# VisionDepth/VisionDepth3D

Hardware: AMD Instinct MI355X
Metric: stereo-pairs/sec end-to-end (depth+warp+fill+mux) (higher is better)
Workload: dtype f32; 1 GPU; 4k-dav2b-dibr; frame=3840x2160, format=Half-SBS, depth_model=depth-anything-v2-base, depth_net_dtype=float32 (the reference's precision), pixel_overlap=True, pixel_streams=2, clip_frames_all_ranks=32, params=render_cli.py defaults + dof_strength 2.0, dense DOF order (parity mode)

## Files before the change

include/vd3d.h:

```cpp
#ifndef VD3D_H
#define VD3D_H

#include <stddef.h>
#include <stdint.h>

#ifdef __cplusplus
extern "C" {
#endif

#define VD3D_ABI_VERSION 6

typedef enum vd3d_status {
  VD3D_OK = 0,
  VD3D_E_INVALID = -1,
  VD3D_E_HIP = -2,
  VD3D_E_NOMEM = -3,
  VD3D_E_UNSUPPORTED = -4
} vd3d_status;

typedef enum vd3d_format {
  VD3D_FMT_HALF_SBS = 0,
  VD3D_FMT_FULL_SBS = 1,
  VD3D_FMT_VR = 2,
  VD3D_FMT_ANAGLYPH = 3,
// ... 117 lines not shown

int vd3d_render_frame_blank(vd3d_ctx* ctx, const uint8_t* frame_bgr, const void* depth, int depth_fmt,
                            const vd3d_render_params* p, uint8_t* out_bgr);

int vd3d_shard_begin(vd3d_ctx* ctx, const vd3d_render_params* p, int n_slots);
int vd3d_shard_pixels(vd3d_ctx* ctx, int slot, const vd3d_render_params* p, uint8_t* out_bgr);
int vd3d_shard_pixels_blank(vd3d_ctx* ctx, int slot, const uint8_t* frame_bgr, const vd3d_render_params* p, uint8_t* out_bgr);
int vd3d_set_pixel_overlap(vd3d_ctx* ctx, int enable);
int vd3d_join_pixels(vd3d_ctx* ctx);
int vd3d_wait_pixels(vd3d_ctx* ctx, int slot);

int vd3d_shard2_p0(vd3d_ctx* ctx, const uint8_t* frame_bgr, const vd3d_render_params* p, int* crop_out_dev);
int vd3d_shard2_set_crops(vd3d_ctx* ctx, const int* crops_all_dev, int n);
int vd3d_shard2_p1(vd3d_ctx* ctx, const uint8_t* frame_bgr, const void* depth, int depth_fmt,
                   const vd3d_render_params* p, int step_idx, int slot, float* q_out_dev);
int vd3d_tdf_plane_export(vd3d_ctx* ctx, float* dst_dev, int eye_h, int eye_w);
int vd3d_tdf_plane_import(vd3d_ctx* ctx, const float* src_dev, int eye_h, int eye_w, int valid);
int vd3d_shard2_r1(vd3d_ctx* ctx, const float* q_all_dev, int n);
int vd3d_shard2_p3(vd3d_ctx* ctx, int slot, int step_idx, const vd3d_render_params* p, long long* m_out_dev);
int vd3d_shard2_p1_batch(vd3d_ctx* ctx, const uint8_t* const* frames_bgr, const void* const* depths, int depth_fmt,
                         const vd3d_render_params* p, int step_idx0, int slot0, int n, float* q_out_dev);
int vd3d_shard2_p3_batch(vd3d_ctx* ctx, int slot0, int step_idx0, int n, const vd3d_render_params* p, long long* m_out_dev);
int vd3d_shard2_r2(vd3d_ctx* ctx, const long long* m_all_dev, const int* own_slot_host, const uint8_t* blank_host_or_null, int n,
                   const vd3d_render_params* p);

int vd3d_heal_missing_pixels(vd3d_ctx* ctx, const float* warped_chw, const float* original_chw, const float* edge_mask_or_null,
                             int H, int W, double heal_strength, float* out_chw);

int vd3d_nv12_to_bgr(vd3d_ctx* ctx, const uint8_t* y_plane, long long y_pitch, const uint8_t* uv_plane, long long uv_pitch, int h, int w,
                     uint8_t* out_bgr);
int vd3d_bgr_to_nv12(vd3d_ctx* ctx, const uint8_t* bgr, int h, int w, uint8_t* y_plane, long long y_pitch, uint8_t* uv_plane,
                     long long uv_pitch);

int vd3d_resize_cubic_u8(vd3d_ctx* ctx, const uint8_t* src, int sh, int sw, int cn, uint8_t* dst, int dh, int dw);
int vd3d_resize_area_u8(vd3d_ctx* ctx, const uint8_t* src_bgr, int sh, int sw, uint8_t* dst_bgr, int dh, int dw);
int vd3d_resize_linear_u8(vd3d_ctx* ctx, const uint8_t* src_bgr, int sh, int sw, uint8_t* dst_bgr, int dh, int dw);
int vd3d_format_3d_output(vd3d_ctx* ctx, const uint8_t* left_bgr, const uint8_t* right_bgr, int h, int w, int format, uint8_t* out_bgr);

int vd3d_esr_preprocess(vd3d_ctx* ctx, int dtype, const uint8_t* frame_bgr, long long pitch_bytes, int h, int w, int channels_last,
                        void* out_rgb);
int vd3d_esr_postprocess(vd3d_ctx* ctx, const float* pred_rgb, int h, int w, int channels_last, int cy, int cx, int ch, int cw,
                         uint8_t* out_bgr, long long pitch_bytes);
int vd3d_add_weighted_u8(vd3d_ctx* ctx, const uint8_t* a, double alpha, const uint8_t* b, double beta, double gamma, long long n,
                         uint8_t* out);
int vd3d_rife_preprocess(vd3d_ctx* ctx, int dtype, const uint8_t* frame1_bgr, const uint8_t* frame2_bgr, int h, int w, int channels_last,
                         void* out6);
int vd3d_rife_postprocess(vd3d_ctx* ctx, const float* pred3, int h, int w, int channels_last, uint8_t* out_bgr);

int vd3d_conv3x3_c64_f16(vd3d_ctx* ctx, const void* x_nhwc, int H, int W, const void* w_frag, const float* bias, const float* slope_or_null,
                         void* y_nhwc);
int vd3d_conv3x3_head_f16(vd3d_ctx* ctx, const void* x_nhwc3, int H, int W, const float* w27x64, const float* bias, const float* slope_or_null,
                          void* y_nhwc64);
int vd3d_esr_tail_f32(vd3d_ctx* ctx, const void* t_nhwc64, const void* x_nhwc3, int H, int W, int r, float* out_planar);
int vd3d_conv3x3_dense_f16(vd3d_ctx* ctx, const void* x, int H, int W, int x_stride, int Cin, const void* w_frag, const float* bias, int Cout,
                           float slope, float alpha, const void* r1_or_null, int r1_stride, float beta, const void* r2_or_null, int r2_stride,
                           int up2, void* y, int y_stride, int y_offset);
int vd3d_nhwc_f16_to_planar3_f32(vd3d_ctx* ctx, const void* t_nhwc32, int H, int W, float* out_planar);

int vd3d_depth_handoff(vd3d_ctx* ctx, const float* pred, int B, int ph, int pw, int H, int W, int invert, uint8_t* out_gray);
int vd3d_depth_handoff_form(vd3d_ctx* ctx, const float* pred, int B, int ph, int pw, int H, int W, int invert, uint8_t* out_gray, int form);

int vd3d_tile_gather_cubic_u8(vd3d_ctx* ctx, const uint8_t* frames_bgr, long long pitch_bytes, long long frame_stride_bytes, int B, int H, int W,
                              const int32_t* origins_dev, int n, int ch, int cw, int chs, int cws, uint8_t* out_tiles);
int vd3d_tile_blend_f32(vd3d_ctx* ctx, const float* pred_pool, const int64_t* pred_off_dev, const int32_t* tile_tab_dev, const float* w_pool,
                        int B, int tgt_h, int tgt_w, int tile, int pad, float* out);
int vd3d_depth_normalize_pclip_u8(vd3d_ctx* ctx, const float* planes, int B, int H, int W, float p_lo, float p_hi, int invert, uint8_t* out_gray,
                                  float* lo_hi_dev_or_null);

typedef struct vd3d_letterbox_state {
  int32_t top, bottom;
  int32_t locked_zero, locked_bars;
  int32_t cand_top, cand_bottom, streak;
  int32_t cooldown;
  int32_t have_prev, prev_h, prev_w;
  int32_t reserved;
} vd3d_letterbox_state;
typedef struct vd3d_letterbox_params {
  int32_t min_change, confirm_needed;
  int32_t max_total;
  int32_t cooldown_frames;
} vd3d_letterbox_params;
int vd3d_letterbox_stats(vd3d_ctx* ctx, const uint8_t* frames_bgr, int B, int H, int W, int chain, float* row_mean, float* row_var,
                         uint32_t* row_sat_sum, uint8_t* gray, uint32_t* hist64, uint64_t* mad_sum, float* frame_mean);
int vd3d_canny_u8(vd3d_ctx* ctx, const uint8_t* gray, int B, int H, int W, int low, int high, uint8_t* edges, int32_t* row_counts_or_null);
int vd3d_canny_hysteresis_u8(vd3d_ctx* ctx, const uint8_t* classes, int B, int H, int W, uint8_t* edges, int32_t* row_counts_or_null);
int vd3d_letterbox_track(vd3d_ctx* ctx, const uint8_t* frames_bgr, int B, int H, int W, const vd3d_letterbox_params* params, int32_t* out_bars);
int vd3d_letterbox_state_reset(vd3d_ctx* ctx);
int vd3d_letterbox_state_export(vd3d_ctx* ctx, vd3d_letterbox_state* out, uint32_t* prev_hist64_host_or_null, uint8_t* prev_gray_dev_or_null,
                                long long gray_capacity);
int vd3d_letterbox_state_import(vd3d_ctx* ctx, const vd3d_letterbox_state* in, const uint32_t* prev_hist64_host_or_null,
                                const uint8_t* prev_gray_dev_or_null);
int vd3d_depth_letterbox_fill_u8(vd3d_ctx* ctx, const uint8_t* depth, int B, int H, int W, const int32_t* bars_dev, int bars_stride, uint8_t* out);

typedef enum vd3d_dtype { VD3D_DT_BF16 = 0, VD3D_DT_F32 = 1, VD3D_DT_F16 = 2  } vd3d_dtype;

int vd3d_depth_preprocess(vd3d_ctx* ctx, const uint8_t* frames_bgr, int B, int H, int W, int th, int tw,
                          const float* mean3_host, const float* std3_host, int dtype, void* out_nhwc);
int vd3d_depth_preprocess_form(vd3d_ctx* ctx, const uint8_t* frames_bgr, int B, int H, int W, int th, int tw,
                               const float* mean3_host, const float* std3_host, int dtype, void* out_nhwc, int form);

int vd3d_resize_pil_bicubic_u8(vd3d_ctx* ctx, const uint8_t* src, int B, int H, int W, uint8_t* dst, int h, int w);
int vd3d_depth_preprocess_pil(vd3d_ctx* ctx, const uint8_t* frames_bgr, int B, int H, int W, int mid_h, int mid_w, int th, int tw,
                              const float* mean3_host, const float* std3_host, int dtype, void* out_nhwc);

int vd3d_add_layernorm(vd3d_ctx* ctx, int dtype, const void* x, const void* y_or_null, const void* gamma, const void* beta,
                       float eps, int64_t rows, int cols, void* out_sum, void* out_norm);

enum { VD3D_GEMM_EPI_NONE = 0, VD3D_GEMM_EPI_GELU = 1 };
enum { VD3D_X3_BF16X3 = 0, VD3D_X3_FP16X2 = 1 };
int64_t vd3d_gemm_x3_weight_bytes(int N, int K, int mode);
int vd3d_gemm_x3_pack_weights(vd3d_ctx* ctx, const float* W, int N, int K, int mode, void* image);
int vd3d_gemm_x3(vd3d_ctx* ctx, const float* X, int64_t M, int K, const void* w_image, int N, int mode, const float* bias_or_null, int epilogue, float* Y);
int64_t vd3d_attention_x3_workspace_bytes(int B, int T, int H, int D, int mode);
int vd3d_attention_x3(vd3d_ctx* ctx, const float* qkv, int B, int T, int H, int D, float scale, int mode, void* workspace, int64_t workspace_bytes, float* out);
int vd3d_attention_f32(vd3d_ctx* ctx, const float* qkv, int B, int T, int H, int D, float scale, float* out);
int vd3d_attention_f32_form(vd3d_ctx* ctx, const float* qkv, int B, int T, int H, int D, float scale, float* out, int form);

int64_t vd3d_conv3x3_x2_weight_bytes(int Cin, int Cout);
int vd3d_conv3x3_x2_pack_weights(vd3d_ctx* ctx, const float* W, int Cin, int Cout, void* image);
int vd3d_conv3x3_x2(vd3d_ctx* ctx, const float* X, int B, int H, int W, int Cin, const void* w_image, int Cout, float* Y);
int64_t vd3d_conv3x3_x3_weight_bytes(int Cin, int Cout);
int vd3d_conv3x3_x3_pack_weights(vd3d_ctx* ctx, const float* W, int Cin, int Cout, void* image);
int vd3d_conv3x3_x3(vd3d_ctx* ctx, const float* X, int B, int H, int W, int Cin, const void* w_image, int Cout, float* Y);
int64_t vd3d_conv3x3_s2_x3_weight_bytes(int Cin, int Cout);
int vd3d_conv3x3_s2_x3_pack_weights(vd3d_ctx* ctx, const float* W, int Cin, int Cout, void* image);
int vd3d_conv3x3_s2_x3(vd3d_ctx* ctx, const float* X, int B, int H, int W, int Cin, const void* w_image, int Cout, float* Y);
int64_t vd3d_conv3x3_s1_x2_weight_bytes(int Cin, int Cout);
int vd3d_conv3x3_s1_x2_pack_weights(vd3d_ctx* ctx, const float* W, int Cin, int Cout, void* image);
int vd3d_conv3x3_s1_x2(vd3d_ctx* ctx, const float* X, int B, int H, int W, int Cin, const void* w_image, int Cout, float* Y);
int64_t vd3d_conv3x3_s2_x2_weight_bytes(int Cin, int Cout);
int vd3d_conv3x3_s2_x2_pack_weights(vd3d_ctx* ctx, const float* W, int Cin, int Cout, void* image);
int vd3d_conv3x3_s2_x2(vd3d_ctx* ctx, const float* X, int B, int H, int W, int Cin, const void* w_image, int Cout, float* Y);

enum { VD3D_IFN_K3S1 = 0, VD3D_IFN_K3S2 = 1, VD3D_IFN_T4S2 = 2 };
int64_t vd3d_conv_ifn_weight_bytes(int kind, int Cin, int Cout);
int vd3d_conv_ifn_pack_weights(vd3d_ctx* ctx, int kind, const float* W, int Cin, int Cout, void* image);
int vd3d_conv_ifn(vd3d_ctx* ctx, int kind, const float* X, int B, int H, int W, int x_stride, int Cin, const void* w_image, const float* bias,
                  const float* slope_or_null, int Cout, const float* r_or_null, int r_stride, float* Y, int y_stride, int y_offset);
int vd3d_rife_warp_pack(vd3d_ctx* ctx, const float* x6, const float* state_or_null, int N, int h, int w, int scale, float* out16);
int vd3d_rife_update(vd3d_ctx* ctx, const float* t, int t_stride, int first, int N, int h, int w, int scale, float* state);
int vd3d_rife_blend(vd3d_ctx* ctx, const float* x6, const float* state, int N, int h, int w, float* out);

int vd3d_upsample_bilinear_nhwc(vd3d_ctx* ctx, int dtype, const void* in, void* out, int B, int ih, int iw, int oh, int ow, int C);

int vd3d_nhwc_bias_act_f32(vd3d_ctx* ctx, const float* y, const float* bias_or_null, const float* r1_or_null, const float* r2_or_null, int relu,
                           int64_t n_pix, int C, float* out, float* relu_out_or_null);
int vd3d_upsample_bilinear_bias_nhwc_f32(vd3d_ctx* ctx, const float* in, const float* bias, float* out, int B, int ih, int iw, int oh, int ow, int C);
int vd3d_dpt_head_tail_f32(vd3d_ctx* ctx, const float* y, const float* b2, const float* w3, float b3, float scale, int64_t n_pix, int C, float* out);

int64_t vd3d_dpt_head_conv_weight_bytes(int Cin, int Cout);
int vd3d_dpt_head_conv_pack_weights(vd3d_ctx* ctx, const float* W, int Cin, int Cout, void* image);
int vd3d_dpt_head_conv_f32(vd3d_ctx* ctx, const float* x, const float* b_in, int B, int ih, int iw, int oh, int ow, int Cin, const void* w_image, int Cout,
                           const float* b2_or_null, const float* w3_or_null, float b3, float scale, float* out);

int vd3d_depth_to_space_bias_nhwc_f32(vd3d_ctx* ctx, const float* y, const float* bias_or_null, int B, int H, int W, int s, int C, float* out);

int vd3d_patchify_f32(vd3d_ctx* ctx, const float* x, int B, int th, int tw, int p, float* rows);

typedef enum vd3d_preview {
  VD3D_PREVIEW_INTERLACED = 0,
  VD3D_PREVIEW_HSBS = 1,
  VD3D_PREVIEW_LR_DIFF = 2,
  VD3D_PREVIEW_FEATHER_BLEND = 3,
  VD3D_PREVIEW_RED_BLUE = 4
} vd3d_preview;
int vd3d_preview_image(vd3d_ctx* ctx, int type, const uint8_t* left_bgr, const uint8_t* right_bgr, int h, int w, uint8_t* out_bgr);
int vd3d_preview_heatmap(vd3d_ctx* ctx, int type, const float* shift_map, int h, int w, const uint8_t* lut_bgr_dev, uint8_t* out_bgr);
int vd3d_preview_arrows(vd3d_ctx* ctx, const uint8_t* left_bgr, const float* shift_map, int h, int w, uint8_t* out_bgr);

int vd3d_finish_frame(vd3d_ctx* ctx, const uint8_t* left_bgr, const uint8_t* right_bgr,
                      const float* depth_norm, int eye_h, int eye_w,
                      const vd3d_render_params* p, double focal_depth, int bar_width, int bar_side,
                      uint8_t* out_bgr);
int vd3d_quantiles(vd3d_ctx* ctx, const float* plane, int64_t n, const float* q_host, int nq, float* out_host);
int vd3d_subject_depth(vd3d_ctx* ctx, const float* plane, int H, int W, float* out_host);
int vd3d_detect_black_bars(vd3d_ctx* ctx, const uint8_t* frame_bgr, int h, int w, int* top_host, int* bottom_host);
int vd3d_stream_copy(vd3d_ctx* ctx, const void* src, void* dst, size_t bytes);
int vd3d_torch_math(vd3d_ctx* ctx, int op, const float* x, float param, float* out, long long n);
int vd3d_torch_math_aten(vd3d_ctx* ctx, int op, const float* x, double param, float* out, long long n, int aten_threads);
int vd3d_set_profiling(vd3d_ctx* ctx, int enable);
int vd3d_debug_tune(int which, int value);
float vd3d_last_stage_ms(vd3d_ctx* ctx, const char* stage);
long vd3d_stage_calls(vd3d_ctx* ctx, const char* stage);
int vd3d_debug_gaussian_kernel1d(int k, float sigma, float* out_host);
int vd3d_debug_exp_torch(const float* x_host, float* out_host, long long n);
int vd3d_debug_planes(vd3d_ctx* ctx, float** D, float** S, uint8_t** L, uint8_t** R, float** rgb_eye, float** dn_cur);

#ifdef __cplusplus
}
#endif
#endif
```

visiondepth3d_amd/_lib.py:

```python
from __future__ import annotations

import ctypes as C
import os

from . import _abi
from ._abi import FrameScalars, LetterboxParams, LetterboxState, RenderParams, ShiftParams, State

_HERE = os.path.dirname(os.path.abspath(__file__))
LIB_PATH = os.environ.get("VD3D_LIB_PATH") or os.path.join(_HERE, "libvd3d_hip.so")

EXPORTS = (
    "vd3d_abi_version", "vd3d_last_error", "vd3d_shift_params_default", "vd3d_render_params_default",
    "vd3d_ctx_create", "vd3d_ctx_destroy", "vd3d_sync", "vd3d_ctx_stream", "vd3d_ctx_set_stream", "vd3d_ctx_pixel_stream", "vd3d_ctx_pixel_stream_k",
    "vd3d_state_reset", "vd3d_state_new_clip", "vd3d_state_export", "vd3d_state_import", "vd3d_state_planes",
    "vd3d_last_scalars", "vd3d_pixel_shift", "vd3d_render_frame", "vd3d_render_frame_blank", "vd3d_depth_handoff", "vd3d_depth_handoff_form", "vd3d_heal_missing_pixels", "vd3d_preview_heatmap", "vd3d_preview_arrows", "vd3d_conv3x3_c64_f16", "vd3d_conv3x3_head_f16", "vd3d_esr_tail_f32", "vd3d_conv3x3_dense_f16", "vd3d_nhwc_f16_to_planar3_f32", "vd3d_nv12_to_bgr", "vd3d_bgr_to_nv12", "vd3d_resize_cubic_u8", "vd3d_resize_area_u8", "vd3d_resize_linear_u8", "vd3d_format_3d_output", "vd3d_esr_preprocess", "vd3d_esr_postprocess", "vd3d_add_weighted_u8", "vd3d_rife_preprocess", "vd3d_rife_postprocess",
    "vd3d_shard_begin", "vd3d_shard_pixels", "vd3d_shard_pixels_blank", "vd3d_tdf_plane_export", "vd3d_tdf_plane_import", "vd3d_set_pixel_overlap", "vd3d_join_pixels", "vd3d_wait_pixels", "vd3d_finish_frame", "vd3d_quantiles",
    "vd3d_subject_depth", "vd3d_shard2_p0", "vd3d_shard2_set_crops", "vd3d_shard2_p1", "vd3d_shard2_p1_batch", "vd3d_shard2_r1", "vd3d_shard2_p3", "vd3d_shard2_p3_batch", "vd3d_shard2_r2", "vd3d_depth_preprocess", "vd3d_depth_preprocess_form", "vd3d_resize_pil_bicubic_u8", "vd3d_depth_preprocess_pil", "vd3d_tile_gather_cubic_u8", "vd3d_tile_blend_f32", "vd3d_depth_normalize_pclip_u8", "vd3d_letterbox_stats", "vd3d_canny_u8", "vd3d_canny_hysteresis_u8", "vd3d_letterbox_track", "vd3d_letterbox_state_reset", "vd3d_letterbox_state_export", "vd3d_letterbox_state_import", "vd3d_depth_letterbox_fill_u8", "vd3d_add_layernorm", "vd3d_gemm_x3_weight_bytes", "vd3d_gemm_x3_pack_weights", "vd3d_gemm_x3", "vd3d_attention_x3_workspace_bytes", "vd3d_attention_x3", "vd3d_attention_f32", "vd3d_attention_f32_form", "vd3d_conv3x3_x2_weight_bytes", "vd3d_conv3x3_x2_pack_weights", "vd3d_conv3x3_x2", "vd3d_conv3x3_x3_weight_bytes", "vd3d_conv3x3_x3_pack_weights", "vd3d_conv3x3_x3", "vd3d_conv3x3_s2_x3_weight_bytes", "vd3d_conv3x3_s2_x3_pack_weights", "vd3d_conv3x3_s2_x3", "vd3d_conv3x3_s1_x2_weight_bytes", "vd3d_conv3x3_s1_x2_pack_weights", "vd3d_conv3x3_s1_x2", "vd3d_conv3x3_s2_x2_weight_bytes", "vd3d_conv3x3_s2_x2_pack_weights", "vd3d_conv3x3_s2_x2", "vd3d_conv_ifn_weight_bytes", "vd3d_conv_ifn_pack_weights", "vd3d_conv_ifn", "vd3d_rife_warp_pack", "vd3d_rife_update", "vd3d_rife_blend", "vd3d_upsample_bilinear_nhwc", "vd3d_nhwc_bias_act_f32", "vd3d_upsample_bilinear_bias_nhwc_f32", "vd3d_dpt_head_tail_f32", "vd3d_dpt_head_conv_weight_bytes", "vd3d_dpt_head_conv_pack_weights", "vd3d_dpt_head_conv_f32", "vd3d_depth_to_space_bias_nhwc_f32", "vd3d_patchify_f32", "vd3d_preview_image", "vd3d_detect_black_bars", "vd3d_stream_copy", "vd3d_torch_math", "vd3d_torch_math_aten", "vd3d_debug_gaussian_kernel1d", "vd3d_debug_exp_torch", "vd3d_set_profiling", "vd3d_last_stage_ms", "vd3d_stage_calls",
    "vd3d_debug_planes", "vd3d_debug_tune",
)

_lib = None


class Vd3dError(RuntimeError):
    def __init__(self, code, msg):
        super().__init__(f"libvd3d_hip error {code}: {msg}")
        self.code = code


def lib():
    global _lib
    if _lib is not None:
        return _lib
    if not os.path.exists(LIB_PATH):
        raise ImportError(f"{LIB_PATH} not built: run `python -c 'import __graft_entry__ as g; g.build()'` "
                          "(hipcc --offload-arch=gfx950). There is no CPU fallback.")
    L = C.CDLL(LIB_PATH)
    vp, i32, f32p, u8p = C.c_void_p, C.c_int, C.c_void_p, C.c_void_p
    L.vd3d_abi_version.restype = i32
    L.vd3d_last_error.restype = C.c_char_p
    L.vd3d_ctx_create.argtypes = [i32, vp, C.POINTER(vp)]
    L.vd3d_ctx_destroy.argtypes = [vp]
    L.vd3d_sync.argtypes = [vp]
    L.vd3d_ctx_stream.argtypes = [vp]
    L.vd3d_ctx_stream.restype = vp
    L.vd3d_ctx_set_stream.argtypes = [vp, vp]
    L.vd3d_ctx_pixel_stream.argtypes = [vp]
    L.vd3d_ctx_pixel_stream.restype = vp
    L.vd3d_ctx_pixel_stream_k.argtypes = [vp, i32]
    L.vd3d_ctx_pixel_stream_k.restype = vp
    for n in ("vd3d_state_reset", "vd3d_state_new_clip"):
        getattr(L, n).argtypes = [vp]
    L.vd3d_state_export.argtypes = [vp, C.POINTER(State)]
    L.vd3d_state_import.argtypes = [vp, C.POINTER(State)]
    L.vd3d_state_planes.argtypes = [vp, C.POINTER(vp), C.POINTER(vp), C.POINTER(i32), C.POINTER(i32)]
    L.vd3d_last_scalars.argtypes = [vp, C.POINTER(FrameScalars)]
    L.vd3d_pixel_shift.argtypes = [vp, f32p, f32p, i32, i32, i32, i32, C.POINTER(ShiftParams), u8p, u8p, f32p]
    L.vd3d_render_frame.argtypes = [vp, u8p, vp, i32, C.POINTER(RenderParams), u8p]
    L.vd3d_render_frame_blank.argtypes = [vp, u8p, vp, i32, C.POINTER(RenderParams), u8p]
    L.vd3d_shard_begin.argtypes = [vp, C.POINTER(RenderParams), i32]
    L.vd3d_shard_pixels.argtypes = [vp, i32, C.POINTER(RenderParams), u8p]
    L.vd3d_shard_pixels_blank.argtypes = [vp, i32, u8p, C.POINTER(RenderParams), u8p]
    L.vd3d_tdf_plane_export.argtypes = [vp, f32p, i32, i32]
    L.vd3d_tdf_plane_import.argtypes = [vp, f32p, i32, i32, i32]
    L.vd3d_set_pixel_overlap.argtypes = [vp, i32]
    L.vd3d_join_pixels.argtypes = [vp]
    L.vd3d_wait_pixels.argtypes = [vp, i32]
    L.vd3d_depth_handoff.argtypes = [vp, f32p, i32, i32, i32, i32, i32, i32, u8p]
    L.vd3d_depth_handoff_form.argtypes = [vp, f32p, i32, i32, i32, i32, i32, i32, u8p, i32]
    L.vd3d_heal_missing_pixels.argtypes = [vp, f32p, f32p, f32p, i32, i32, C.c_double, f32p]
    L.vd3d_resize_cubic_u8.argtypes = [vp, u8p, i32, i32, i32, u8p, i32, i32]
    L.vd3d_nv12_to_bgr.argtypes = [vp, u8p, C.c_longlong, u8p, C.c_longlong, i32, i32, u8p]
    L.vd3d_bgr_to_nv12.argtypes = [vp, u8p, i32, i32, u8p, C.c_longlong, u8p, C.c_longlong]
    L.vd3d_conv3x3_c64_f16.argtypes = [vp, vp, i32, i32, vp, vp, vp, vp]
    L.vd3d_conv3x3_head_f16.argtypes = [vp, vp, i32, i32, vp, vp, vp, vp]
    L.vd3d_esr_tail_f32.argtypes = [vp, vp, vp, i32, i32, i32, vp]
    L.vd3d_conv3x3_dense_f16.argtypes = [vp, vp, i32, i32, i32, i32, vp, vp, i32, C.c_float, C.c_float, vp, i32, C.c_float, vp, i32, i32, vp, i32, i32]
    L.vd3d_nhwc_f16_to_planar3_f32.argtypes = [vp, vp, i32, i32, vp]
    L.vd3d_preview_arrows.argtypes = [vp, u8p, f32p, i32, i32, u8p]
    L.vd3d_preview_heatmap.argtypes = [vp, i32, f32p, i32, i32, u8p, u8p]
    L.vd3d_resize_area_u8.argtypes = [vp, u8p, i32, i32, u8p, i32, i32]
    L.vd3d_resize_linear_u8.argtypes = [vp, u8p, i32, i32, u8p, i32, i32]
    L.vd3d_format_3d_output.argtypes = [vp, u8p, u8p, i32, i32, i32, u8p]
    L.vd3d_esr_preprocess.argtypes = [vp, i32, u8p, C.c_longlong, i32, i32, i32, vp]
    L.vd3d_esr_postprocess.argtypes = [vp, f32p, i32, i32, i32, i32, i32, i32, i32, u8p, C.c_longlong]
    L.vd3d_rife_preprocess.argtypes = [vp, i32, u8p, u8p, i32, i32, i32, vp]
    L.vd3d_rife_postprocess.argtypes = [vp, f32p, i32, i32, i32, u8p]
    L.vd3d_add_weighted_u8.argtypes = [vp, u8p, C.c_double, u8p, C.c_double, C.c_double, C.c_longlong, u8p]
    L.vd3d_finish_frame.argtypes = [vp, u8p, u8p, f32p, i32, i32, C.POINTER(RenderParams), C.c_double, i32, i32, u8p]
    L.vd3d_quantiles.argtypes = [vp, f32p, C.c_int64, C.POINTER(C.c_float), i32, C.POINTER(C.c_float)]
    L.vd3d_subject_depth.argtypes = [vp, f32p, i32, i32, C.POINTER(C.c_float)]
    L.vd3d_shard2_p0.argtypes = [vp, vp, vp, vp]
    L.vd3d_shard2_set_crops.argtypes = [vp, vp, i32]
    L.vd3d_shard2_p1.argtypes = [vp, vp, vp, i32, vp, i32, i32, vp]
    L.vd3d_shard2_p1_batch.argtypes = [vp, vp, vp, i32, vp, i32, i32, i32, vp]
    L.vd3d_shard2_p3_batch.argtypes = [vp, i32, i32, i32, vp, vp]
    L.vd3d_shard2_r1.argtypes = [vp, vp, i32]
    L.vd3d_shard2_p3.argtypes = [vp, i32, i32, vp, vp]
    L.vd3d_shard2_r2.argtypes = [vp, vp, C.POINTER(C.c_int), C.POINTER(C.c_uint8), i32, vp]
    L.vd3d_depth_preprocess.argtypes = [vp, vp, i32, i32, i32, i32, i32, C.POINTER(C.c_float), C.POINTER(C.c_float), i32, vp]
    L.vd3d_depth_preprocess_form.argtypes = [vp, vp, i32, i32, i32, i32, i32, C.POINTER(C.c_float), C.POINTER(C.c_float), i32, vp, i32]
    L.vd3d_resize_pil_bicubic_u8.argtypes = [vp, u8p, i32, i32, i32, u8p, i32, i32]
    L.vd3d_depth_preprocess_pil.argtypes = [vp, vp, i32, i32, i32, i32, i32, i32, i32, C.POINTER(C.c_float), C.POINTER(C.c_float), i32, vp]
    L.vd3d_tile_gather_cubic_u8.argtypes = [vp, u8p, C.c_longlong, C.c_longlong, i32, i32, i32, vp, i32, i32, i32, i32, i32, u8p]
    L.vd3d_tile_blend_f32.argtypes = [vp, f32p, vp, vp, f32p, i32, i32, i32, i32, i32, f32p]
    L.vd3d_depth_normalize_pclip_u8.argtypes = [vp, f32p, i32, i32, i32, C.c_float, C.c_float, i32, u8p, f32p]
    L.vd3d_letterbox_stats.argtypes = [vp, u8p, i32, i32, i32, i32, f32p, f32p, vp, u8p, vp, vp, f32p]
    L.vd3d_canny_u8.argtypes = [vp, u8p, i32, i32, i32, i32, i32, u8p, vp]
    L.vd3d_canny_hysteresis_u8.argtypes = [vp, u8p, i32, i32, i32, u8p, vp]
    L.vd3d_letterbox_track.argtypes = [vp, u8p, i32, i32, i32, C.POINTER(LetterboxParams), vp]
    L.vd3d_letterbox_state_reset.argtypes = [vp]
    L.vd3d_letterbox_state_export.argtypes = [vp, C.POINTER(LetterboxState), vp, u8p, C.c_longlong]
    L.vd3d_letterbox_state_import.argtypes = [vp, C.POINTER(LetterboxState), vp, u8p]
    L.vd3d_depth_letterbox_fill_u8.argtypes = [vp, u8p, i32, i32, i32, vp, i32, u8p]
    L.vd3d_gemm_x3_weight_bytes.argtypes = [i32, i32, i32]
    L.vd3d_gemm_x3_weight_bytes.restype = C.c_int64
    L.vd3d_gemm_x3_pack_weights.argtypes = [vp, vp, i32, i32, i32, vp]
    L.vd3d_gemm_x3.argtypes = [vp, vp, C.c_int64, i32, vp, i32, i32, vp, i32, vp]
    L.vd3d_attention_x3_workspace_bytes.argtypes = [i32, i32, i32, i32, i32]
    L.vd3d_attention_x3_workspace_bytes.restype = C.c_int64
    L.vd3d_attention_x3.argtypes = [vp, vp, i32, i32, i32, i32, C.c_float, i32, vp, C.c_int64, vp]
    L.vd3d_attention_f32.argtypes = [vp, vp, i32, i32, i32, i32, C.c_float, vp]
    L.vd3d_attention_f32_form.argtypes = [vp, vp, i32, i32, i32, i32, C.c_float, vp, i32]
    L.vd3d_conv3x3_x2_weight_bytes.argtypes = [i32, i32]
    L.vd3d_conv3x3_x2_weight_bytes.restype = C.c_int64
    L.vd3d_conv3x3_x2_pack_weights.argtypes = [vp, vp, i32, i32, vp]
    L.vd3d_conv3x3_x2.argtypes = [vp, vp, i32, i32, i32, i32, vp, i32, vp]
    L.vd3d_conv3x3_x3_weight_bytes.argtypes = [i32, i32]
    L.vd3d_conv3x3_x3_weight_bytes.restype = C.c_int64
    L.vd3d_conv3x3_x3_pack_weights.argtypes = [vp, vp, i32, i32, vp]
    L.vd3d_conv3x3_x3.argtypes = [vp, vp, i32, i32, i32, i32, vp, i32, vp]
    L.vd3d_conv3x3_s2_x3_weight_bytes.argtypes = [i32, i32]
    L.vd3d_conv3x3_s2_x3_weight_bytes.restype = C.c_int64
    L.vd3d_conv3x3_s2_x3_pack_weights.argtypes = [vp, vp, i32, i32, vp]
    L.vd3d_conv3x3_s2_x3.argtypes = [vp, vp, i32, i32, i32, i32, vp, i32, vp]
    for st in ("s1", "s2"):
        getattr(L, f"vd3d_conv3x3_{st}_x2_weight_bytes").argtypes = [i32, i32]
        getattr(L, f"vd3d_conv3x3_{st}_x2_weight_bytes").restype = C.c_int64
        getattr(L, f"vd3d_conv3x3_{st}_x2_pack_weights").argtypes = [vp, vp, i32, i32, vp]
        getattr(L, f"vd3d_conv3x3_{st}_x2").argtypes = [vp, vp, i32, i32, i32, i32, vp, i32, vp]
    L.vd3d_conv_ifn_weight_bytes.argtypes = [i32, i32, i32]
    L.vd3d_conv_ifn_weight_bytes.restype = C.c_int64
    L.vd3d_conv_ifn_pack_weights.argtypes = [vp, i32, vp, i32, i32, vp]
    L.vd3d_conv_ifn.argtypes = [vp, i32, vp, i32, i32, i32, i32, i32, vp, vp, vp, i32, vp, i32, vp, i32, i32]
    L.vd3d_rife_warp_pack.argtypes = [vp, vp, vp, i32, i32, i32, i32, vp]
    L.vd3d_rife_update.argtypes = [vp, vp, i32, i32, i32, i32, i32, i32, vp]
    L.vd3d_rife_blend.argtypes = [vp, vp, vp, i32, i32, i32, vp]
    L.vd3d_add_layernorm.argtypes = [vp, i32, vp, vp, vp, vp, C.c_float, C.c_int64, i32, vp, vp]
    L.vd3d_upsample_bilinear_nhwc.argtypes = [vp, i32, vp, vp, i32, i32, i32, i32, i32, i32]
    L.vd3d_nhwc_bias_act_f32.argtypes = [vp, vp, vp, vp, vp, i32, C.c_int64, i32, vp, vp]
    L.vd3d_upsample_bilinear_bias_nhwc_f32.argtypes = [vp, vp, vp, vp, i32, i32, i32, i32, i32, i32]
    L.vd3d_dpt_head_tail_f32.argtypes = [vp, vp, vp, vp, C.c_float, C.c_float, C.c_int64, i32, vp]
    L.vd3d_dpt_head_conv_weight_bytes.argtypes = [i32, i32]
    L.vd3d_dpt_head_conv_weight_bytes.restype = C.c_int64
    L.vd3d_dpt_head_conv_pack_weights.argtypes = [vp, vp, i32, i32, vp]
    L.vd3d_dpt_head_conv_f32.argtypes = [vp, vp, vp, i32, i32, i32, i32, i32, i32, vp, i32, vp, vp, C.c_float, C.c_float, vp]
    L.vd3d_depth_to_space_bias_nhwc_f32.argtypes = [vp, vp, vp, i32, i32, i32, i32, i32, vp]
    L.vd3d_patchify_f32.argtypes = [vp, vp, i32, i32, i32, i32, vp]
    L.vd3d_preview_image.argtypes = [vp, i32, vp, vp, i32, i32, vp]
    L.vd3d_detect_black_bars.argtypes = [vp, vp, i32, i32, C.POINTER(C.c_int), C.POINTER(C.c_int)]
    L.vd3d_stream_copy.argtypes = [vp, vp, vp, C.c_size_t]
    L.vd3d_torch_math.argtypes = [vp, i32, vp, C.c_float, vp, C.c_longlong]
    L.vd3d_torch_math_aten.argtypes = [vp, i32, vp, C.c_double, vp, C.c_longlong, i32]
    L.vd3d_debug_gaussian_kernel1d.argtypes = [i32, C.c_float, vp]
    L.vd3d_debug_exp_torch.argtypes = [vp, vp, C.c_longlong]
    L.vd3d_debug_tune.argtypes = [i32, i32]
    L.vd3d_set_profiling.argtypes = [vp, i32]
    L.vd3d_last_stage_ms.argtypes = [vp, C.c_char_p]
    L.vd3d_last_stage_ms.restype = C.c_float
    L.vd3d_stage_calls.argtypes = [vp, C.c_char_p]
    L.vd3d_stage_calls.restype = C.c_long
    L.vd3d_debug_planes.argtypes = [vp] + [C.POINTER(vp)] * 6
    L.vd3d_shift_params_default.argtypes = [C.POINTER(ShiftParams)]
    L.vd3d_render_params_default.argtypes = [C.POINTER(RenderParams)]
    if L.vd3d_abi_version() != _abi.ABI_VERSION:
        raise ImportError("libvd3d_hip.so ABI version mismatch")
    if os.environ.get("VD3D_TUNE"):
        if L.vd3d_debug_tune(-1, 0) != 0:
            raise ImportError("VD3D_TUNE is set but this libvd3d_hip.so was built without -DVD3D_DEV_KNOBS (bash tools/build_ab.sh dev -DVD3D_DEV_KNOBS; VD3D_LIB_PATH=...)")
        for kv in filter(None, os.environ["VD3D_TUNE"].split(",")):
            k, v = kv.split(":")
            if L.vd3d_debug_tune(int(k), int(v)) != 0:
                raise ImportError(f"VD3D_TUNE: unknown knob {k}")
    _lib = L
    return L


def check(rc):
    if rc != 0:
        raise Vd3dError(rc, lib().vd3d_last_error().decode(errors="replace"))
```

visiondepth3d_amd/csrc/vd3d_api.hip:

```cpp
#include <hip/hip_runtime.h>

#include <cmath>
#include <cstdarg>
#include <cstddef>
#include <cstdio>
#include <cstring>
#include <cstdlib>
#include <list>
#include <map>
#include <string>
#include <vector>

#include "vd3d_kernels.h"

#define VD3D_EXPORT extern "C" __attribute__((visibility("default")))

static thread_local char g_err[512] = "";
static int set_err(int code, const char* fmt, ...) {
  va_list ap;
  va_start(ap, fmt);
  vsnprintf(g_err, sizeof g_err, fmt, ap);
  va_end(ap);
  return code;
}
// ... 1693 lines not shown
    return set_err(VD3D_E_UNSUPPORTED, "conv_ifn: bias, slope, residual and output must be 4-byte aligned");
  const int Ho = kind == VD3D_IFN_K3S2 ? (H + 1) / 2 : kind == VD3D_IFN_T4S2 ? 2 * H : H, Wo = kind == VD3D_IFN_K3S2 ? (W + 1) / 2 : kind == VD3D_IFN_T4S2 ? 2 * W : W;
  {
    const long long in_pix = (long long)B * H * W, out_pix = (long long)B * Ho * Wo;
    const uintptr_t xb = (uintptr_t)X, xe = xb + (uintptr_t)(((in_pix - 1) * x_stride + Cin) * 4);
    const uintptr_t yb = (uintptr_t)Y + (uintptr_t)y_offset * 4, ye = (uintptr_t)Y + (uintptr_t)(((out_pix - 1) * y_stride + y_offset + Cout) * 4);
    const bool same_grid = (const void*)X == (const void*)Y && x_stride == y_stride && kind == VD3D_IFN_K3S1;
    if (same_grid ? y_offset < Cin : (xb < ye && yb < xe))
      return set_err(VD3D_E_UNSUPPORTED, "conv_ifn: the output slice [%d, %d) meets the input channels [0, %d) of the same buffer (a race between workgroups)",
                     y_offset, y_offset + Cout, Cin);
    if (r_or_null) {
      const uintptr_t rb = (uintptr_t)r_or_null, re = rb + (uintptr_t)(((out_pix - 1) * r_stride + Cout) * 4);
      const bool rgrid = (const void*)r_or_null == (const void*)Y && r_stride == y_stride;
      if (rgrid ? y_offset < Cout : (rb < ye && yb < re)) return set_err(VD3D_E_UNSUPPORTED, "conv_ifn: the residual overlaps the output slice");
    }
  }
  HIPCHK(hipSetDevice(c->device));
  StageTimer t(c, "conv_ifn");
  if (!vd_launch_conv_ifn(c->stream, kind, X, B, H, W, x_stride, Cin, w_image, bias, slope_or_null, Cout, r_or_null, r_stride, Y, y_stride, y_offset))
    return set_err(VD3D_E_HIP, "conv_ifn: the dynamic LDS opt-in failed");
  HIPCHK(hipGetLastError());
  return 0;
}

static int rife_glue_err(const char* what, int N, int h, int w, int scale) {
  return set_err(VD3D_E_UNSUPPORTED, "%s: N %d must be 1 .. 65535, the frame %d x %d 1 .. 32768 on each side, scale %d one of 1, 2, 4 and every pointer 16-byte aligned", what, N, h, w, scale);
}
static bool rife_glue_ok(int N, int h, int w, int scale) { return N >= 1 && N <= 65535 && h >= 1 && w >= 1 && h <= 32768 && w <= 32768 && (scale == 1 || scale == 2 || scale == 4); }

VD3D_EXPORT int vd3d_rife_warp_pack(vd3d_ctx* c, const float* x6, const float* state_or_null, int N, int h, int w, int scale, float* out16) {
  if (!c || !x6 || !out16) return set_err(VD3D_E_INVALID, "rife_warp_pack: null argument");
  if (!rife_glue_ok(N, h, w, scale) || (((uintptr_t)x6 | (uintptr_t)state_or_null | (uintptr_t)out16) & 15)) return rife_glue_err("rife_warp_pack", N, h, w, scale);
  HIPCHK(hipSetDevice(c->device));
  StageTimer t(c, "rife_glue");
  vd_launch_rife_warp_pack(c->stream, x6, state_or_null, state_or_null ? 0 : 1, N, h, w, (h + 31) / 32 * 32, (w + 31) / 32 * 32, scale, out16);
  HIPCHK(hipGetLastError());
  return 0;
}

VD3D_EXPORT int vd3d_rife_update(vd3d_ctx* c, const float* t_, int t_stride, int first, int N, int h, int w, int scale, float* state) {
  if (!c || !t_ || !state) return set_err(VD3D_E_INVALID, "rife_update: null argument");
  if (!rife_glue_ok(N, h, w, scale) || (((uintptr_t)t_ | (uintptr_t)state) & 15)) return rife_glue_err("rife_update", N, h, w, scale);
  if (t_stride < 5 || (t_stride & 3)) return set_err(VD3D_E_UNSUPPORTED, "rife_update: t_stride %d must be a multiple of 4 and >= 5", t_stride);
  HIPCHK(hipSetDevice(c->device));
  StageTimer t(c, "rife_glue");
  vd_launch_rife_update(c->stream, t_, t_stride, first ? 1 : 0, N, (h + 31) / 32 * 32, (w + 31) / 32 * 32, scale, state);
  HIPCHK(hipGetLastError());
  return 0;
}

VD3D_EXPORT int vd3d_rife_blend(vd3d_ctx* c, const float* x6, const float* state, int N, int h, int w, float* out) {
  if (!c || !x6 || !state || !out) return set_err(VD3D_E_INVALID, "rife_blend: null argument");
  if (!rife_glue_ok(N, h, w, 1) || (((uintptr_t)x6 | (uintptr_t)state | (uintptr_t)out) & 15)) return rife_glue_err("rife_blend", N, h, w, 1);
  HIPCHK(hipSetDevice(c->device));
  StageTimer t(c, "rife_glue");
  vd_launch_rife_blend(c->stream, x6, state, N, h, w, (h + 31) / 32 * 32, (w + 31) / 32 * 32, out);
  HIPCHK(hipGetLastError());
  return 0;
}

VD3D_EXPORT int64_t vd3d_attention_x3_workspace_bytes(int B, int T, int H, int D, int mode) { return (int64_t)vd_attn_x3_workspace_bytes(B, T, H, D, mode); }

VD3D_EXPORT int vd3d_attention_x3(vd3d_ctx* c, const float* qkv, int B, int T, int H, int D, float scale, int mode, void* workspace, int64_t workspace_bytes, float* out) {
  if (!c || !qkv || !workspace || !out) return set_err(VD3D_E_INVALID, "bad argument");
  const long long need = vd_attn_x3_workspace_bytes(B, T, H, D, mode);
  if (need < 0) return set_err(VD3D_E_UNSUPPORTED, "attention_x3: head size %d not built (64), an unknown mode %d or an empty shape (B %d T %d H %d)", D, mode, B, T, H);
  if (workspace_bytes < need) return set_err(VD3D_E_INVALID, "attention_x3: workspace of %lld bytes, %lld needed", (long long)workspace_bytes, need);
  HIPCHK(hipSetDevice(c->device));
  if (!vd_launch_attn_x3(c->stream, qkv, B, T, H, D, scale, workspace, out, mode))
    return set_err(VD3D_E_UNSUPPORTED, "attention_x3: qkv / workspace / out must be 16-byte aligned, B * H <= 65535");
  HIPCHK(hipGetLastError());
  return 0;
}

VD3D_EXPORT int vd3d_attention_f32_form(vd3d_ctx* c, const float* qkv, int B, int T, int H, int D, float scale, float* out, int form) {
  if (!c || !qkv || !out) return set_err(VD3D_E_INVALID, "bad argument");
  if (form != 0 && form != 4 && form != 8) return set_err(VD3D_E_INVALID, "attention_f32: form %d is not 0 (choose), 4 or 8 waves per workgroup", form);
  HIPCHK(hipSetDevice(c->device));
  if (!vd_launch_attn_f32(c->stream, qkv, B, T, H, D, scale, out, form))
    return set_err(VD3D_E_UNSUPPORTED, "attention_f32: head size %d not built (64), an empty shape (B %d T %d H %d), B * H > 65535 or qkv / out not 16-byte aligned", D, B, T, H);
  HIPCHK(hipGetLastError());
  return 0;
}

VD3D_EXPORT int vd3d_attention_f32(vd3d_ctx* c, const float* qkv, int B, int T, int H, int D, float scale, float* out) {
  return vd3d_attention_f32_form(c, qkv, B, T, H, D, scale, out, 0);
}

VD3D_EXPORT int64_t vd3d_gemm_x3_weight_bytes(int N, int K, int mode) { return (int64_t)vd_gemm_x3_weight_bytes(N, K, mode); }

VD3D_EXPORT int vd3d_gemm_x3_pack_weights(vd3d_ctx* c, const float* W, int N, int K, int mode, void* image) {
  if (!c || !W || !image) return set_err(VD3D_E_INVALID, "bad argument");
  HIPCHK(hipSetDevice(c->device));
  if (!vd_launch_gemm_x3_pack_w(c->stream, W, N, K, image, mode)) return set_err(VD3D_E_UNSUPPORTED, "gemm_x3: K %d must be a positive multiple of 16 (N %d), mode %d in {0, 1}", K, N, mode);
  HIPCHK(hipGetLastError());
  return 0;
}

VD3D_EXPORT int vd3d_gemm_x3(vd3d_ctx* c, const float* X, int64_t M, int K, const void* w_image, int N, int mode, const float* bias_or_null, int epilogue, float* Y) {
  if (!c || !X || !w_image || !Y || M < 1) return set_err(VD3D_E_INVALID, "bad argument");
  if (epilogue != VD3D_GEMM_EPI_NONE && epilogue != VD3D_GEMM_EPI_GELU) return set_err(VD3D_E_INVALID, "gemm_x3: unknown epilogue %d", epilogue);
  HIPCHK(hipSetDevice(c->device));
  if (!vd_launch_gemm_x3(c->stream, X, (long long)M, K, w_image, N, bias_or_null, epilogue, Y, mode))
    return set_err(VD3D_E_UNSUPPORTED, "gemm_x3: K %d must be a positive multiple of 16, mode %d in {0, 1}, X and the weight image 16-byte aligned", K, mode);
  HIPCHK(hipGetLastError());
  return 0;
}

VD3D_EXPORT int vd3d_upsample_bilinear_nhwc(vd3d_ctx* c, int dtype, const void* in, void* out, int B, int ih, int iw, int oh, int ow, int C) {
  if (dtype != VD3D_DT_BF16 && dtype != VD3D_DT_F32) return set_err(VD3D_E_INVALID, "bad dtype %d", dtype);
  if (!c || !in || !out || B < 1 || ih < 1 || iw < 1) return set_err(VD3D_E_INVALID, "bad argument");
  if (!vd_launch_upsample_bilinear_nhwc(c->stream, dtype, in, out, B, ih, iw, oh, ow, C))
    return set_err(VD3D_E_UNSUPPORTED, "upsample_bilinear_nhwc: C not a multiple of 8 (bf16) / 4 (f32) or output smaller than 2x2");
  HIPCHK(hipGetLastError());
  return 0;
}

VD3D_EXPORT int vd3d_nhwc_bias_act_f32(vd3d_ctx* c, const float* y, const float* bias_or_null, const float* r1_or_null, const float* r2_or_null, int relu,
                                       int64_t n_pix, int C, float* out, float* relu_out_or_null) {
  if (!c || !y || !out || n_pix < 1 || C < 4) return set_err(VD3D_E_INVALID, "bad argument");
  HIPCHK(hipSetDevice(c->device));
  if (!vd_launch_bias_act_f32(c->stream, y, bias_or_null, r1_or_null, r2_or_null, relu, (long long)n_pix, C, out, relu_out_or_null))
    return set_err(VD3D_E_UNSUPPORTED, "nhwc_bias_act: C %d not a multiple of 4", C);
  HIPCHK(hipGetLastError());
  return 0;
}
VD3D_EXPORT int vd3d_upsample_bilinear_bias_nhwc_f32(vd3d_ctx* c, const float* in, const float* bias, float* out, int B, int ih, int iw, int oh, int ow, int C) {
  if (!c || !in || !bias || !out || B < 1 || ih < 1 || iw < 1) return set_err(VD3D_E_INVALID, "bad argument");
  HIPCHK(hipSetDevice(c->device));
  if (!vd_launch_upsample_bilinear_bias_nhwc_f32(c->stream, in, bias, out, B, ih, iw, oh, ow, C))
    return set_err(VD3D_E_UNSUPPORTED, "upsample_bilinear_bias_nhwc: C not a multiple of 4 or output smaller than 2x2");
  HIPCHK(hipGetLastError());
  return 0;
}
VD3D_EXPORT int vd3d_dpt_head_tail_f32(vd3d_ctx* c, const float* y, const float* b2, const float* w3, float b3, float scale, int64_t n_pix, int C, float* out) {
  if (!c || !y || !b2 || !w3 || !out || n_pix < 1) return set_err(VD3D_E_INVALID, "bad argument");
  HIPCHK(hipSetDevice(c->device));
  if (!vd_launch_head_tail_f32(c->stream, y, b2, w3, b3, scale, (long long)n_pix, C, out))
    return set_err(VD3D_E_UNSUPPORTED, "dpt_head_tail: C %d not in {16, 32, 64}", C);
  HIPCHK(hipGetLastError());
  return 0;
}
VD3D_EXPORT int64_t vd3d_dpt_head_conv_weight_bytes(int Cin, int Cout) { return (int64_t)vd_dpt_head_conv_weight_bytes(Cin, Cout); }
VD3D_EXPORT int vd3d_dpt_head_conv_pack_weights(vd3d_ctx* c, const float* W, int Cin, int Cout, void* image) {
  if (!c || !W || !image) return set_err(VD3D_E_INVALID, "bad argument");
  if (vd_dpt_head_conv_weight_bytes(Cin, Cout) < 0)
    return set_err(VD3D_E_UNSUPPORTED, "dpt_head_conv: shape not built: %d -> %d channels (built: 32 | 64 | 128 -> 32 with the tail, 128 -> 64 plain)", Cin, Cout);
  if (reinterpret_cast<uintptr_t>(image) & 15) return set_err(VD3D_E_UNSUPPORTED, "dpt_head_conv: the weight image must be 16-byte aligned");
  HIPCHK(hipSetDevice(c->device));
  if (!vd_launch_dpt_head_conv_pack(c->stream, W, Cin, Cout, image)) return set_err(VD3D_E_HIP, "dpt_head_conv: the weight pack launch failed");
  HIPCHK(hipGetLastError());
  return 0;
}
VD3D_EXPORT int vd3d_dpt_head_conv_f32(vd3d_ctx* c, const float* x, const float* b_in, int B, int ih, int iw, int oh, int ow, int Cin, const void* w_image, int Cout,
                                       const float* b2_or_null, const float* w3_or_null, float b3, float scale, float* out) {
  if (!c || !x || !b_in || !w_image || !out || (b2_or_null == nullptr) != (w3_or_null == nullptr)) return set_err(VD3D_E_INVALID, "bad argument");
  const bool tail = b2_or_null != nullptr;
  if (!vd_dpt_head_conv_shape_ok(B, ih, iw, oh, ow, Cin, Cout, tail))
    return set_err(VD3D_E_UNSUPPORTED, "dpt_head_conv: shape not built: %d -> %d channels %s, batch %d, %d x %d -> %d x %d (built: 32 | 64 | 128 -> 32 with the tail, "
                   "128 -> 64 plain; batch 1 .. 65535; output at least 2 x 2; a frame below 2^31 elements)", Cin, Cout, tail ? "with the tail" : "plain", B, ih, iw, oh, ow);
  if ((reinterpret_cast<uintptr_t>(x) & 15) || (reinterpret_cast<uintptr_t>(b_in) & 15) || (reinterpret_cast<uintptr_t>(w_image) & 15) ||
      (reinterpret_cast<uintptr_t>(out) & (tail ? 3 : 15)) || (tail && ((reinterpret_cast<uintptr_t>(b2_or_null) & 15) || (reinterpret_cast<uintptr_t>(w3_or_null) & 15))))
    return set_err(VD3D_E_UNSUPPORTED, "dpt_head_conv: x, b_in, the weight image, b2, w3 and a plain output must be 16-byte aligned (the tail's output 4-byte)");
  HIPCHK(hipSetDevice(c->device));
  if (!vd_launch_dpt_head_conv_f32(c->stream, x, b_in, B, ih, iw, oh, ow, Cin, w_image, Cout, b2_or_null, w3_or_null, b3, scale, out))
    return set_err(VD3D_E_HIP, "dpt_head_conv: the dynamic LDS opt-in or the launch failed");
  HIPCHK(hipGetLastError());
  return 0;
}
VD3D_EXPORT int vd3d_depth_to_space_bias_nhwc_f32(vd3d_ctx* c, const float* y, const float* bias_or_null, int B, int H, int W, int s, int C, float* out) {
  if (!c || !y || !out || B < 1 || H < 1 || W < 1 || s < 1 || C < 1) return set_err(VD3D_E_INVALID, "bad argument");
  HIPCHK(hipSetDevice(c->device));
  if (!vd_launch_depth_to_space_bias_f32(c->stream, y, bias_or_null, B, H, W, s, C, out))
    return set_err(VD3D_E_UNSUPPORTED, "depth_to_space_bias: C %d not a multiple of 4, y / bias / out not 16-byte aligned, or a map too large for one grid", C);
  HIPCHK(hipGetLastError());
  return 0;
}
VD3D_EXPORT int vd3d_patchify_f32(vd3d_ctx* c, const float* x, int B, int th, int tw, int p, float* out) {
  if (!c || !x || !out) return set_err(VD3D_E_INVALID, "bad argument");
  if (B < 1 || p < 1 || p > 64 || th < p || tw < p)
    return set_err(VD3D_E_UNSUPPORTED, "patchify: batch %d must be at least 1, the patch size %d 1 .. 64 and the image %d x %d at least one patch", B, p, th, tw);
  if ((reinterpret_cast<uintptr_t>(x) & 3) || (reinterpret_cast<uintptr_t>(out) & 15))
    return set_err(VD3D_E_UNSUPPORTED, "patchify: the rows must be 16-byte aligned (the image 4-byte)");
  HIPCHK(hipSetDevice(c->device));
  if (!vd_launch_patchify_f32(c->stream, x, B, th, tw, p, out)) return set_err(VD3D_E_UNSUPPORTED, "patchify: too many rows for one grid");
  HIPCHK(hipGetLastError());
  return 0;
}

VD3D_EXPORT int vd3d_preview_image(vd3d_ctx* c, int type, const uint8_t* left_bgr, const uint8_t* right_bgr, int h, int w, uint8_t* out_bgr) {
  if (!c || !left_bgr || !right_bgr || !out_bgr || h < 1 || w < 1) return set_err(VD3D_E_INVALID, "bad argument");
  HIPCHK(hipSetDevice(c->device));
  if (!vd_launch_preview(c->stream, type, left_bgr, right_bgr, h, w, out_bgr))
    return set_err(VD3D_E_UNSUPPORTED, "preview type %d (colour-mapped heat-maps / arrow overlay need OpenCV's tables and rasteriser)", type);
  HIPCHK(hipGetLastError());
  return 0;
}

VD3D_EXPORT int vd3d_preview_heatmap(vd3d_ctx* c, int type, const float* shift_map, int h, int w, const uint8_t* lut_bgr_dev, uint8_t* out_bgr) {
  if (!c || !shift_map || !lut_bgr_dev || !out_bgr || h < 1 || w < 1) return set_err(VD3D_E_INVALID, "bad argument");
  HIPCHK(hipSetDevice(c->device));
  if (c->mm_cap < 1) { HIPCHK(re_alloc(&c->mm, (size_t)3)); c->mm_cap = 1; }
  if (!vd_launch_preview_heatmap(c->stream, type, shift_map, h, w, lut_bgr_dev, c->mm, out_bgr))
    return set_err(VD3D_E_UNSUPPORTED, "heat-map type %d (0 shift, 1 |shift|, 2 clipped, 3 feather mask)", type);
  HIPCHK(hipGetLastError());
  return 0;
}

VD3D_EXPORT int vd3d_conv3x3_c64_f16(vd3d_ctx* c, const void* x_nhwc, int H, int W, const void* w_frag, const float* bias, const float* slope_or_null,
                                     void* y_nhwc) {
  if (!c || !x_nhwc || !w_frag || !bias || !y_nhwc || H < 1 || W < 1 || x_nhwc == y_nhwc) return set_err(VD3D_E_INVALID, "bad argument");
  if ((long long)H * W * 128 >= (1ll << 32)) return set_err(VD3D_E_INVALID, "conv3x3_c64_f16: activation larger than 4 GB");
  if (((uintptr_t)x_nhwc | (uintptr_t)y_nhwc | (uintptr_t)w_frag | (uintptr_t)bias | (uintptr_t)slope_or_null) & 15)
    return set_err(VD3D_E_INVALID, "conv3x3_c64_f16: pointers must be 16-byte aligned");
  HIPCHK(hipSetDevice(c->device));
  StageTimer t(c, "conv3x3");
  if (!vd_launch_conv3x3_c64_f16(c->stream, x_nhwc, H, W, w_frag, bias, slope_or_null, y_nhwc)) return set_err(VD3D_E_HIP, "conv3x3_c64_f16: LDS attribute");
  HIPCHK(hipGetLastError());
  return 0;
}

VD3D_EXPORT int vd3d_conv3x3_head_f16(vd3d_ctx* c, const void* x_nhwc3, int H, int W, const float* w27x64, const float* bias, const float* slope_or_null,
                                      void* y_nhwc64) {
  if (!c || !x_nhwc3 || !w27x64 || !bias || !y_nhwc64 || H < 1 || W < 1) return set_err(VD3D_E_INVALID, "conv3x3_head_f16: bad argument");
  if ((long long)H * W * 128 >= (1ll << 32)) return set_err(VD3D_E_INVALID, "conv3x3_head_f16: activation larger than 4 GB");
  if ((reinterpret_cast<uintptr_t>(y_nhwc64) | reinterpret_cast<uintptr_t>(w27x64)) & 15) return set_err(VD3D_E_INVALID, "conv3x3_head_f16: y and w must be 16-byte aligned");
  HIPCHK(hipSetDevice(c->device));
  StageTimer t(c, "conv_head");
  vd_launch_conv3x3_head_f16(c->stream, x_nhwc3, H, W, w27x64, bias, slope_or_null, y_nhwc64);
  HIPCHK(hipGetLastError());
  return 0;
}

VD3D_EXPORT int vd3d_esr_tail_f32(vd3d_ctx* c, const void* t_nhwc64, const void* x_nhwc3, int H, int W, int r, float* out_planar) {
  if (!c || !t_nhwc64 || !x_nhwc3 || !out_planar || H < 1 || W < 1 || (r != 2 && r != 4)) return set_err(VD3D_E_INVALID, "esr_tail_f32: bad argument (r = 2 or 4)");
  if (reinterpret_cast<uintptr_t>(t_nhwc64) & 15) return set_err(VD3D_E_INVALID, "esr_tail_f32: t must be 16-byte aligned");
  HIPCHK(hipSetDevice(c->device));
  StageTimer t(c, "esr_tail");
  vd_launch_esr_tail_f32(c->stream, t_nhwc64, x_nhwc3, H, W, r, out_planar);
  HIPCHK(hipGetLastError());
  return 0;
}

VD3D_EXPORT int vd3d_conv3x3_dense_f16(vd3d_ctx* c, const void* x, int H, int W, int x_stride, int Cin, const void* w_frag, const float* bias, int Cout,
                                       float slope, float alpha, const void* r1_or_null, int r1_stride, float beta, const void* r2_or_null, int r2_stride,
                                       int up2, void* y, int y_stride, int y_offset) {
  if (!c || !x || !w_frag || !bias || !y) return set_err(VD3D_E_INVALID, "conv3x3_dense_f16: null argument");
  if (H < 1 || W < 1 || H > 32768 || W > 32768) return set_err(VD3D_E_UNSUPPORTED, "conv3x3_dense_f16: map %d x %d must be 1 .. 32768 on each side", H, W);
  if (Cin != 64 && Cin != 96 && Cin != 128 && Cin != 160 && Cin != 192)
    return set_err(VD3D_E_UNSUPPORTED, "conv3x3_dense_f16: C_in %d must be one of 64, 96, 128, 160, 192", Cin);
  if (Cout != 32 && Cout != 64) return set_err(VD3D_E_UNSUPPORTED, "conv3x3_dense_f16: C_out %d must be 32 or 64", Cout);
  if (x_stride < Cin || (x_stride & 7)) return set_err(VD3D_E_UNSUPPORTED, "conv3x3_dense_f16: x_stride %d must be a multiple of 8 and >= C_in %d", x_stride, Cin);
  if (y_offset < 0 || (y_offset & 7) || (y_stride & 7) || y_stride < y_offset + Cout)
    return set_err(VD3D_E_UNSUPPORTED, "conv3x3_dense_f16: y_offset %d and y_stride %d must be multiples of 8 with y_offset + C_out %d <= y_stride", y_offset, y_stride, Cout);
  if ((r1_or_null && (r1_stride < Cout || (r1_stride & 7))) || (r2_or_null && (r2_stride < Cout || (r2_stride & 7))))
    return set_err(VD3D_E_UNSUPPORTED, "conv3x3_dense_f16: a residual's stride must be a multiple of 8 and >= C_out %d", Cout);
  if (up2 && (Cin != 64 || Cout != 64 || (H & 1) || (W & 1)))
    return set_err(VD3D_E_UNSUPPORTED, "conv3x3_dense_f16: up2 is built for 64 -> 64 channels and an even output size (got %d -> %d, %d x %d)", Cin, Cout, H, W);
  if (((uintptr_t)x | (uintptr_t)y | (uintptr_t)w_frag | (uintptr_t)bias | (uintptr_t)r1_or_null | (uintptr_t)r2_or_null) & 15)
    return set_err(VD3D_E_UNSUPPORTED, "conv3x3_dense_f16: pointers must be 16-byte aligned");
  const long long in_pix = up2 ? (long long)(H / 2) * (W / 2) : (long long)H * W, out_pix = (long long)H * W;
  {
    const uintptr_t xb = (uintptr_t)x, xe = xb + (uintptr_t)(((in_pix - 1) * x_stride + Cin) * 2);
    const uintptr_t yb = (uintptr_t)y + (uintptr_t)y_offset * 2, ye = (uintptr_t)y + (uintptr_t)(((out_pix - 1) * y_stride + y_offset + Cout) * 2);
    const bool same_grid = x == y && x_stride == y_stride && !up2;
    if (same_grid ? y_offset < Cin : (xb < ye && yb < xe))
      return set_err(VD3D_E_UNSUPPORTED, "conv3x3_dense_f16: the output slice [%d, %d) meets the input channels [0, %d) of the same buffer (a race between workgroups)",
                     y_offset, y_offset + Cout, Cin);
    const void* rs[2] = {r1_or_null, r2_or_null};
    const int rst[2] = {r1_stride, r2_stride};
    for (int i = 0; i < 2; ++i) {
      if (!rs[i]) continue;
      const uintptr_t rb = (uintptr_t)rs[i], re = rb + (uintptr_t)(((out_pix - 1) * rst[i] + Cout) * 2);
      const bool rgrid = rs[i] == y && rst[i] == y_stride;
      if (rgrid ? y_offset < Cout : (rb < ye && yb < re))
        return set_err(VD3D_E_UNSUPPORTED, "conv3x3_dense_f16: residual %d overlaps the output slice", i + 1);
    }
  }
  HIPCHK(hipSetDevice(c->device));
  StageTimer t(c, "conv3x3_dense");
  if (!vd_launch_conv3x3_dense_f16(c->stream, x, H, W, x_stride, Cin, w_frag, bias, Cout, slope, alpha, r1_or_null, r1_stride, beta, r2_or_null, r2_stride,
                                   up2 ? 1 : 0, y, y_stride, y_offset))
    return set_err(VD3D_E_HIP, "conv3x3_dense_f16: the dynamic LDS opt-in failed");
  HIPCHK(hipGetLastError());
  return 0;
}

VD3D_EXPORT int vd3d_nhwc_f16_to_planar3_f32(vd3d_ctx* c, const void* t_nhwc32, int H, int W, float* out_planar) {
  if (!c || !t_nhwc32 || !out_planar) return set_err(VD3D_E_INVALID, "nhwc_f16_to_planar3_f32: null argument");
  if (H < 1 || W < 1 || H > 32768 || W > 32768) return set_err(VD3D_E_UNSUPPORTED, "nhwc_f16_to_planar3_f32: map %d x %d must be 1 .. 32768 on each side", H, W);
  if (((uintptr_t)t_nhwc32 & 15) || ((uintptr_t)out_planar & 3)) return set_err(VD3D_E_UNSUPPORTED, "nhwc_f16_to_planar3_f32: t must be 16-byte and out 4-byte aligned");
  HIPCHK(hipSetDevice(c->device));
  StageTimer t(c, "esr_tail");
  vd_launch_nhwc_f16_to_planar3_f32(c->stream, t_nhwc32, H, W, out_planar);
  HIPCHK(hipGetLastError());
  return 0;
}

VD3D_EXPORT int vd3d_nv12_to_bgr(vd3d_ctx* c, const uint8_t* y_plane, long long y_pitch, const uint8_t* uv_plane, long long uv_pitch, int h, int w,
                                 uint8_t* out_bgr) {
  if (!c || !y_plane || !uv_plane || !out_bgr || h < 2 || w < 2 || (h & 1) || (w & 1) || y_pitch < w || uv_pitch < w)
    return set_err(VD3D_E_INVALID, "bad argument (NV12 needs even h and w)");
  HIPCHK(hipSetDevice(c->device));
  StageTimer t(c, "nv12_in");
  vd_launch_nv12_to_bgr(c->stream, y_plane, uv_plane, h, w, y_pitch, uv_pitch, out_bgr);
  HIPCHK(hipGetLastError());
  return 0;
}
VD3D_EXPORT int vd3d_bgr_to_nv12(vd3d_ctx* c, const uint8_t* bgr, int h, int w, uint8_t* y_plane, long long y_pitch, uint8_t* uv_plane,
                                 long long uv_pitch) {
  if (!c || !y_plane || !uv_plane || !bgr || h < 2 || w < 2 || (h & 1) || (w & 1) || y_pitch < w || uv_pitch < w)
    return set_err(VD3D_E_INVALID, "bad argument (NV12 needs even h and w)");
  HIPCHK(hipSetDevice(c->device));
  StageTimer t(c, "nv12_out");
  vd_launch_bgr_to_nv12(c->stream, bgr, h, w, y_plane, uv_plane, y_pitch, uv_pitch);
  HIPCHK(hipGetLastError());
  return 0;
}

VD3D_EXPORT int vd3d_preview_arrows(vd3d_ctx* c, const uint8_t* left_bgr, const float* shift_map, int h, int w, uint8_t* out_bgr) {
  if (!c || !left_bgr || !shift_map || !out_bgr || h < 1 || w < 1 || left_bgr == out_bgr) return set_err(VD3D_E_INVALID, "bad argument");
// ... 86 lines not shown
```

visiondepth3d_amd/csrc/vd3d_conv_head.hip:

```cpp
#include "vd3d_dev.h"
#include "vd3d_kernels.h"
#include "vd3d_x3.h"

typedef float ch_f4 __attribute__((ext_vector_type(4)));

#define CH_TH 8
#define CH_TW 32
#define CH_PW (CH_TW + 2)
#define CH_NPIX ((CH_TH + 2) * CH_PW)
#define CH_NT 512
#define CH_PLANE 388
#define CH_X_BUF (4 * CH_PLANE * 16)
#define CH_ITEMS (CH_NPIX * 4)
#define CH_ITERS ((CH_ITEMS + CH_NT - 1) / CH_NT)
__host__ __device__ constexpr int ch_w_buf(int cout) { return 9 * 4 * cout * 16; }
__host__ __device__ constexpr int ch_w_lds(int cout) { return (ch_w_buf(cout) + CH_NT * 16 - 1) / (CH_NT * 16) * (CH_NT * 16); }
__host__ __device__ constexpr int ch_lds(int cout) { return 2 * CH_X_BUF + 2 * ch_w_lds(cout); }
static_assert(ch_lds(32) == 98816 && ch_lds(64) == 131584 && ch_lds(64) <= 163840 && CH_PLANE * 4 >= CH_ITERS * CH_NT && CH_ITERS == 3, "LDS plan");

struct vd_ch_args {
  int ih, iw, oh, ow;
  float sh, sw;
  int ntx;
  float b3, scale;
};

template <int C_IN, int C_OUT, bool TAIL>
__global__ __launch_bounds__(CH_NT) void k_conv3x3_up_f32(const float* __restrict__ X, const float* __restrict__ bin, const float* __restrict__ Wimg,
                                                          const float* __restrict__ b2, const float* __restrict__ w3, float* __restrict__ out, vd_ch_args a) {
  constexpr int NM = C_OUT / 32, NCHUNK = C_IN / 16, WBUF = ch_w_buf(C_OUT), WLDS = ch_w_lds(C_OUT), W_ITEMS = WBUF / 16, W_ITERS = (W_ITEMS + CH_NT - 1) / CH_NT;
  extern __shared__ __attribute__((aligned(16))) uint8_t ch_smem[];
  const int tile = blockIdx.x, b = blockIdx.y;
  const int tyi = tile / a.ntx, txi = tile - tyi * a.ntx;
  const int y0 = tyi * CH_TH, x0 = txi * CH_TW;
  const int tid = threadIdx.x, lane = tid & 63, wave = __builtin_amdgcn_readfirstlane(tid >> 6);
  const int li = lane & 31, kh = lane >> 5;
  const float* xb = X + (size_t)b * a.ih * a.iw * C_IN;

  int o00[CH_ITERS], o01[CH_ITERS], o10[CH_ITERS], o11[CH_ITERS], dst[CH_ITERS];
  float ly1[CH_ITERS], lx1[CH_ITERS];
  bool inside[CH_ITERS];
#pragma unroll
  for (int it = 0; it < CH_ITERS; ++it) {
    const int i = it * CH_NT + tid, pix = i >> 2, q = i & 3;
    const int py = pix / CH_PW, px = pix - py * CH_PW;
    const int gy = y0 - 1 + py, gx = x0 - 1 + px;
    inside[it] = i < CH_ITEMS && gy >= 0 && gy < a.oh && gx >= 0 && gx < a.ow;
    const int cy = inside[it] ? gy : 0, cx = inside[it] ? gx : 0;
    const float fy = a.sh * (float)cy, fx = a.sw * (float)cx;
    const int yy0 = (int)fy, xx0 = (int)fx;
    const int yy1 = yy0 + (yy0 < a.ih - 1 ? 1 : 0), xx1 = xx0 + (xx0 < a.iw - 1 ? 1 : 0);
    ly1[it] = fy - (float)yy0; lx1[it] = fx - (float)xx0;
    o00[it] = (yy0 * a.iw + xx0) * C_IN + q * 4; o01[it] = (yy0 * a.iw + xx1) * C_IN + q * 4;
    o10[it] = (yy1 * a.iw + xx0) * C_IN + q * 4; o11[it] = (yy1 * a.iw + xx1) * C_IN + q * 4;
    dst[it] = (q * CH_PLANE + pix) * 16;
  }
  ch_f4 p00[CH_ITERS], p01[CH_ITERS], p10[CH_ITERS], p11[CH_ITERS], wv[W_ITERS], bq;
  auto load = [&](int chunk) {
#pragma unroll
    for (int it = 0; it < CH_ITERS; ++it) {
      p00[it] = *reinterpret_cast<const ch_f4*>(xb + o00[it] + chunk * 16); p01[it] = *reinterpret_cast<const ch_f4*>(xb + o01[it] + chunk * 16);
      p10[it] = *reinterpret_cast<const ch_f4*>(xb + o10[it] + chunk * 16); p11[it] = *reinterpret_cast<const ch_f4*>(xb + o11[it] + chunk * 16);
    }
    bq = *reinterpret_cast<const ch_f4*>(bin + chunk * 16 + (tid & 3) * 4);
#pragma unroll
    for (int p = 0; p < W_ITERS; ++p)
      wv[p] = *reinterpret_cast<const ch_f4*>(Wimg + (size_t)chunk * (WBUF / 4) + (p * CH_NT + tid < W_ITEMS ? p * CH_NT + tid : W_ITEMS - 1) * 4);
  };
  auto interp = [&](int it, int buf) {
    asm volatile("" : "+v"(p00[it]), "+v"(p01[it]), "+v"(p10[it]), "+v"(p11[it]));
    const float l_y1 = ly1[it], l_y0 = 1.f - l_y1, l_x1 = lx1[it], l_x0 = 1.f - l_x1;
    ch_f4 o;
    o.x = (l_y0 * (l_x0 * p00[it].x + l_x1 * p01[it].x) + l_y1 * (l_x0 * p10[it].x + l_x1 * p11[it].x)) + bq.x;
    o.y = (l_y0 * (l_x0 * p00[it].y + l_x1 * p01[it].y) + l_y1 * (l_x0 * p10[it].y + l_x1 * p11[it].y)) + bq.y;
    o.z = (l_y0 * (l_x0 * p00[it].z + l_x1 * p01[it].z) + l_y1 * (l_x0 * p10[it].z + l_x1 * p11[it].z)) + bq.z;
    o.w = (l_y0 * (l_x0 * p00[it].w + l_x1 * p01[it].w) + l_y1 * (l_x0 * p10[it].w + l_x1 * p11[it].w)) + bq.w;
    if (!inside[it]) o = ch_f4{0.f, 0.f, 0.f, 0.f};
    *reinterpret_cast<ch_f4*>(ch_smem + buf * CH_X_BUF + dst[it]) = o;
  };
  auto put_w = [&](int buf) {
#pragma unroll
    for (int p = 0; p < W_ITERS; ++p) *reinterpret_cast<ch_f4*>(ch_smem + 2 * CH_X_BUF + buf * WLDS + (p * CH_NT + tid) * 16) = wv[p];
  };

  x3_f16 tot[NM];
#pragma unroll
  for (int m = 0; m < NM; ++m)
#pragma unroll
    for (int r = 0; r < 16; ++r) tot[m][r] = 0.f;

  load(0);
#pragma unroll
  for (int it = 0; it < CH_ITERS; ++it) interp(it, 0);
  put_w(0);
  __syncthreads();

  const int fx_base = (kh * CH_PLANE + (wave + 1) * CH_PW + li + 1) * 16;
  const int fw_base = 2 * CH_X_BUF + (kh * C_OUT + li) * 16;
#pragma unroll 1
  for (int chunk = 0; chunk < NCHUNK; ++chunk) {
    const int cur = chunk & 1, nxt = cur ^ 1;
    load(chunk + 1 < NCHUNK ? chunk + 1 : chunk);
    __builtin_amdgcn_sched_barrier(0);
    const uint8_t* xs = ch_smem + cur * CH_X_BUF + fx_base;
    const uint8_t* ws = ch_smem + cur * WLDS + fw_base;
    x3_f16 acc[2][NM];
#pragma unroll
    for (int m = 0; m < NM; ++m)
#pragma unroll
      for (int r = 0; r < 16; ++r) acc[0][m][r] = acc[1][m][r] = 0.f;
#pragma unroll
    for (int tap = 0; tap < 9; ++tap) {
      const int dy = tap / 3 - 1, dx = tap - (tap / 3) * 3 - 1;
#pragma unroll
      for (int g = 0; g < 2; ++g) {
        const ch_f4 bf = *reinterpret_cast<const ch_f4*>(xs + (2 * g * CH_PLANE + dy * CH_PW + dx) * 16);
        ch_f4 af[NM];
#pragma unroll
        for (int m = 0; m < NM; ++m) af[m] = *reinterpret_cast<const ch_f4*>(ws + ((tap * 4 + 2 * g) * C_OUT + m * 32) * 16);
#pragma unroll
        for (int m = 0; m < NM; ++m) acc[0][m] = __builtin_amdgcn_mfma_f32_32x32x2f32(af[m].x, bf.x, acc[0][m], 0, 0, 0);
#pragma unroll
        for (int m = 0; m < NM; ++m) acc[1][m] = __builtin_amdgcn_mfma_f32_32x32x2f32(af[m].y, bf.y, acc[1][m], 0, 0, 0);
#pragma unroll
        for (int m = 0; m < NM; ++m) acc[0][m] = __builtin_amdgcn_mfma_f32_32x32x2f32(af[m].z, bf.z, acc[0][m], 0, 0, 0);
#pragma unroll
        for (int m = 0; m < NM; ++m) acc[1][m] = __builtin_amdgcn_mfma_f32_32x32x2f32(af[m].w, bf.w, acc[1][m], 0, 0, 0);
      }
      if (tap == 2 || tap == 4 || tap == 6 || tap == 7) __builtin_amdgcn_sched_barrier(0);
      if (tap == 2) interp(0, nxt);
      if (tap == 4) interp(1, nxt);
      if (tap == 6) interp(2, nxt);
      if (tap == 7) put_w(nxt);
    }
#pragma unroll
    for (int m = 0; m < NM; ++m) tot[m] = (tot[m] + acc[0][m]) + acc[1][m];
    __syncthreads();
  }

  const int y = y0 + wave, x = x0 + li;
  const bool live = y < a.oh && x < a.ow;
  const size_t pix = ((size_t)b * a.oh + (live ? y : 0)) * a.ow + (live ? x : 0);
  if constexpr (TAIL) {
    float s = 0.f;
#pragma unroll
    for (int g4 = 0; g4 < 4; ++g4) {
      const ch_f4 bb = *reinterpret_cast<const ch_f4*>(b2 + 8 * g4 + 4 * kh), ww = *reinterpret_cast<const ch_f4*>(w3 + 8 * g4 + 4 * kh);
      s = vd_fma(fmaxf(tot[0][4 * g4] + bb.x, 0.f), ww.x, s);
      s = vd_fma(fmaxf(tot[0][4 * g4 + 1] + bb.y, 0.f), ww.y, s);
      s = vd_fma(fmaxf(tot[0][4 * g4 + 2] + bb.z, 0.f), ww.z, s);
      s = vd_fma(fmaxf(tot[0][4 * g4 + 3] + bb.w, 0.f), ww.w, s);
    }
    s += __shfl_xor(s, 32, 64);
    if (live && kh == 0) out[pix] = fmaxf(s + a.b3, 0.f) * a.scale;
  } else {
    if (live) {
#pragma unroll
      for (int m = 0; m < NM; ++m)
#pragma unroll
        for (int g4 = 0; g4 < 4; ++g4)
          *reinterpret_cast<ch_f4*>(out + pix * C_OUT + m * 32 + 8 * g4 + 4 * kh) =
              ch_f4{tot[m][4 * g4], tot[m][4 * g4 + 1], tot[m][4 * g4 + 2], tot[m][4 * g4 + 3]};
    }
  }
}

__global__ __launch_bounds__(256) void k_conv3x3_up_pack(const float* __restrict__ W, int Cout, int Cin, float4* __restrict__ img) {
  const int t = blockIdx.x * 256 + threadIdx.x;
  const int total = (Cin / 16) * 9 * 4 * Cout;
  if (t >= total) return;
  const int oc = t % Cout, q = (t / Cout) & 3, tap = (t / (4 * Cout)) % 9, chunk = t / (36 * Cout);
  const float* w = W + ((size_t)oc * Cin + chunk * 16 + q * 4) * 9 + tap;
  img[t] = make_float4(w[0], w[9], w[18], w[27]);
}

static bool ch_shape_ok(int Cin, int Cout, bool tail) {
  if (tail) return Cout == 32 && (Cin == 32 || Cin == 64 || Cin == 128);
  return Cout == 64 && Cin == 128;
}
long long vd_dpt_head_conv_weight_bytes(int Cin, int Cout) {
  if (!ch_shape_ok(Cin, Cout, true) && !ch_shape_ok(Cin, Cout, false)) return -1;
  return (long long)Cin * 9 * Cout * 4;
}
bool vd_launch_dpt_head_conv_pack(hipStream_t s, const float* W, int Cin, int Cout, void* img) {
  if (vd_dpt_head_conv_weight_bytes(Cin, Cout) < 0 || (reinterpret_cast<uintptr_t>(img) & 15)) return false;
  const int total = (Cin / 16) * 9 * 4 * Cout;
  hipLaunchKernelGGL(k_conv3x3_up_pack, dim3((total + 255) / 256), dim3(256), 0, s, W, Cout, Cin, reinterpret_cast<float4*>(img));
  return true;
}

bool vd_dpt_head_conv_shape_ok(int B, int ih, int iw, int oh, int ow, int Cin, int Cout, bool tail) {
  if (!ch_shape_ok(Cin, Cout, tail) || B < 1 || B > 65535 || ih < 1 || iw < 1 || oh < 2 || ow < 2) return false;
  if ((long long)ih * iw * Cin >= (1ll << 31)) return false;
  if (((long long)(oh + CH_TH - 1) / CH_TH) * ((ow + CH_TW - 1) / CH_TW) >= (1ll << 31)) return false;
  return true;
}

bool vd_launch_dpt_head_conv_f32(hipStream_t s, const float* x, const float* b_in, int B, int ih, int iw, int oh, int ow, int Cin, const void* wimg, int Cout,
                                 const float* b2, const float* w3, float b3, float scale, float* out) {
  const bool tail = b2 != nullptr;
  if (!vd_dpt_head_conv_shape_ok(B, ih, iw, oh, ow, Cin, Cout, tail)) return false;
  static bool attr_set[64] = {};
  if (!vd_lds_optin({{reinterpret_cast<const void*>(k_conv3x3_up_f32<32, 32, true>), ch_lds(32)}, {reinterpret_cast<const void*>(k_conv3x3_up_f32<64, 32, true>), ch_lds(32)},
                     {reinterpret_cast<const void*>(k_conv3x3_up_f32<128, 32, true>), ch_lds(32)}, {reinterpret_cast<const void*>(k_conv3x3_up_f32<128, 64, false>), ch_lds(64)}},
                    attr_set)) return false;
  vd_ch_args a;
  a.ih = ih; a.iw = iw; a.oh = oh; a.ow = ow;
  a.sh = (float)(ih - 1) / (float)(oh - 1); a.sw = (float)(iw - 1) / (float)(ow - 1);
  a.ntx = (ow + CH_TW - 1) / CH_TW;
  a.b3 = b3; a.scale = scale;
  const dim3 grid((unsigned)(a.ntx * ((oh + CH_TH - 1) / CH_TH)), (unsigned)B, 1);
  const float* wi = reinterpret_cast<const float*>(wimg);
  if (!tail) hipLaunchKernelGGL((k_conv3x3_up_f32<128, 64, false>), grid, dim3(CH_NT), ch_lds(64), s, x, b_in, wi, b2, w3, out, a);
  else if (Cin == 32) hipLaunchKernelGGL((k_conv3x3_up_f32<32, 32, true>), grid, dim3(CH_NT), ch_lds(32), s, x, b_in, wi, b2, w3, out, a);
  else if (Cin == 64) hipLaunchKernelGGL((k_conv3x3_up_f32<64, 32, true>), grid, dim3(CH_NT), ch_lds(32), s, x, b_in, wi, b2, w3, out, a);
  else hipLaunchKernelGGL((k_conv3x3_up_f32<128, 32, true>), grid, dim3(CH_NT), ch_lds(32), s, x, b_in, wi, b2, w3, out, a);
  return true;
}
```

visiondepth3d_amd/csrc/vd3d_kernels.h:

```cpp
#pragma once
#include <hip/hip_runtime.h>

#include <initializer_list>
#include <mutex>

#include "vd3d_work.h"

struct vd_lds_fn { const void* fn; int bytes; };
inline bool vd_lds_optin(std::initializer_list<vd_lds_fn> fns, bool (&done)[64]) {
  static std::mutex mu;
  int dev = 0;
  if (hipGetDevice(&dev) != hipSuccess || dev < 0 || dev >= 64) return false;
  std::lock_guard<std::mutex> lock(mu);
  if (!done[dev]) {
    for (const vd_lds_fn& f : fns)
      if (hipFuncSetAttribute(f.fn, hipFuncAttributeMaxDynamicSharedMemorySize, f.bytes) != hipSuccess) return false;
    done[dev] = true;
  }
  return true;
}

enum { VD_ST_A0 = 0, VD_ST_B0, VD_ST_A1, VD_ST_B1, VD_ST_A2, VD_ST_B2,
       VD_ST_AQ, VD_ST_BQ, VD_ST_BS };
#define PL_KMAX_HOST 129
// ... 49 lines not shown
#include "vd3d_dev.h"
VD_DEV float vd_curved_depth(const float* __restrict__ dn, int ih, int iw, int H, int W, int y, int x) {
  float d;
  if (ih == H && iw == W) {
    d = dn[(size_t)y * W + x];
  } else {
    vd_tap ty = vd_interp_tap(ih, H, y), tx = vd_interp_tap(iw, W, x);
    const float* r0 = dn + (size_t)ty.i0 * iw;
    const float* r1 = dn + (size_t)ty.i1 * iw;
    d = vd_bilerp(r0[tx.i0], r0[tx.i1], r1[tx.i0], r1[tx.i1], tx.w0, tx.w1, ty.w0, ty.w1);
  }
  const float xx = vd_lin11(W, x), yy = vd_lin11(H, y);
  const float curv = 1.f - (xx * xx + yy * yy);
  return vd_clamp(d + curv * (float)0.08, 0.f, 1.f);
}

VD_DEV float vd_depth_at(const void* depth, int fmt, size_t idx) {
  if (fmt == VD3D_DEPTH_F32) return ((const float*)depth)[idx];
  if (fmt == VD3D_DEPTH_GRAY_U8) return vd_u8_unit((float)((const uint8_t*)depth)[idx]);
  const uint8_t* p = (const uint8_t*)depth + idx * 3;
  int g = (p[0] * 1868 + p[1] * 9617 + p[2] * 4899 + 8192) >> 14;
  return vd_u8_unit((float)g);
}
VD_DEV float vd_ingest_pixel(const uint8_t* __restrict__ frame, const void* __restrict__ depth, int fmt, const vd3d_render_params& p,
                             int tdf_valid, float* __restrict__ rgb_eye, const float* tdf_prev, float* tdf, int ey, int ex) {
  const vd_tap ty = vd_interp_tap(p.crop_h, p.eye_h, ey), tx = vd_interp_tap(p.crop_w, p.eye_w, ex);
  const size_t i00 = (size_t)(ty.i0 + p.crop_y) * p.src_w + (tx.i0 + p.crop_x);
  const size_t i01 = (size_t)(ty.i0 + p.crop_y) * p.src_w + (tx.i1 + p.crop_x);
  const size_t i10 = (size_t)(ty.i1 + p.crop_y) * p.src_w + (tx.i0 + p.crop_x);
  const size_t i11 = (size_t)(ty.i1 + p.crop_y) * p.src_w + (tx.i1 + p.crop_x);
  const size_t ne = (size_t)p.eye_h * p.eye_w, o = (size_t)ey * p.eye_w + ex;
  const bool pm_c = vd_interp_premult(3, p.eye_h, p.eye_w, p.aten_sum_threads), pm_d = vd_interp_premult(1, p.eye_h, p.eye_w, p.aten_sum_threads);
  if (frame) {
#pragma unroll
    for (int c = 0; c < 3; ++c) {
      const int sc = 2 - c;
      float p00 = vd_u8_unit((float)frame[i00 * 3 + sc]), p01 = vd_u8_unit((float)frame[i01 * 3 + sc]);
      float p10 = vd_u8_unit((float)frame[i10 * 3 + sc]), p11 = vd_u8_unit((float)frame[i11 * 3 + sc]);
      rgb_eye[c * ne + o] = vd_bilerp_sel(pm_c, p00, p01, p10, p11, tx.w0, tx.w1, ty.w0, ty.w1);
    }
  }
  const float cur = vd_bilerp_sel(pm_d, vd_depth_at(depth, fmt, i00), vd_depth_at(depth, fmt, i01), vd_depth_at(depth, fmt, i10),
                                  vd_depth_at(depth, fmt, i11), tx.w0, tx.w1, ty.w0, ty.w1);
  const float prev = tdf_valid ? tdf_prev[o] : cur;
  const float nv = 0.5f * prev + (float)(1 - 0.5) * cur;
  tdf[o] = nv;
  return nv;
}
#endif

void vd_launch_shard2_r1(hipStream_t s, vd_dev_work* w, const float* q_all, int n, float* etab);
void vd_launch_shard2_r2(hipStream_t s, vd_dev_work* w, const long long* m_all, const float* etab, const int* own_slot_host,
                         const uint8_t* blank_host_or_null, int n, vd_dev_work* slot_work, const vd_stage_args& a);
void vd_launch_autocrop(hipStream_t s, const uint8_t* frame, int h, int wd, double target_ratio, uint32_t* rowflag, vd_dev_work* w,
                        int* crop_out = nullptr);
void vd_set_batch_grid_div(int v);
void vd_launch_chain_eye(hipStream_t s, const vd_batch& b, int fmt, const vd3d_render_params& p, const vd_stage_args& a);
void vd_launch_chain_work(hipStream_t s, const vd_batch& b, int have_eye, int ih, int iw, int H, int W, float mid, float gamma,
                          const vd_stage_args& a);

void vd_launch_hist_eye_d(hipStream_t s, bool passB, const float* tdf, long long n, vd_dev_work* w, uint32_t* histA, uint32_t* histB);
void vd_launch_hist_work_s1(hipStream_t s, bool passB, const float* D, int H, int W, vd_dev_work* w, uint32_t* histA, uint32_t* histB);
void vd_launch_scalar_stage(hipStream_t s, vd_dev_work* w, const uint32_t* histA, const uint32_t* histB, const vd_stage_args& a);

struct vd_finish_consts {
  int nlev;
  int ksz[4];
  float kern[4][32];
  float w2[4][81];
  float fw, imax;
  float sat, con, bri;
  float sharp_kn, sharp_kc;
};
struct vd_shift_consts {
  float mid, fg, mg, bg, fgm, bgm, pb, half_width, fs, ma, mb;
  int edge;
};
vd_shift_consts vd_shift_consts_of(const vd3d_shift_params& p, int W);
void vd_launch_shift(hipStream_t s, const float* D, int H, int W, const vd_dev_work* w, const vd3d_shift_params& p, float* S);
struct vd_shift_fold { const vd_dev_work* work; vd3d_shift_params sp; float* S_out; };
bool vd_warp_fold_ok(int ih, int iw, int H, int W, const vd3d_shift_params& warp_p, const vd3d_shift_params& shift_p);
void vd_launch_e2(hipStream_t s, const float* D, const float* S, int H, int W, float fs, float* e2L, float* e2R);
void vd_launch_pool(hipStream_t s, const float* e2L, const float* e2R, int H, int W, int k, float* bL, float* bR);
void vd_launch_warp(hipStream_t s, const float* rgb, int ih, int iw, const float* S, const float* bL, const float* bR, int H, int W,
                    int feather, uint8_t* L, uint8_t* R);
bool vd_launch_warp_fused(hipStream_t s, const float* rgb, int ih, int iw, const float* D, const float* S, int H, int W,
                          const vd3d_shift_params& p, uint8_t* L, uint8_t* R, const float* E2 = nullptr, const vd_shift_fold* fold = nullptr);
bool vd_warp_fused_ok(int ih, int iw, int H, int W, const vd3d_shift_params& p);
void vd_launch_e2w(hipStream_t s, const float* D, const float* S, int H, int W, float feather_strength, float* E2);
void vd_set_warp_pre_th(int th);
void vd_set_warp_order(int v);
void vd_set_warp_nofeather_th(int th);
#ifdef __cplusplus
#include <vector>
bool vd_aten_plan_build(int eh, int ew, int T, std::vector<int>& pieces_flat, int* n_small, int* n_big, int* nr_crop, int* nr_mad);
#endif
void vd_launch_aten_sums(hipStream_t s, const vd_batch& b, const vd_stage_args& a);
void vd_set_finish_persist(int k);
void vd_set_finish_xcd(int on);
void vd_set_conv_mode(int v);
void vd_launch_dof_grade(hipStream_t s, const uint8_t* eye_in, const float* dn, int eh, int ew, int H, int W,
                         const vd_finish_consts& fc, const vd_dev_work* w, float focal_override, int use_override,
                         int bar_width, int bar_side, uint8_t* eye_out, int dense = 0, const float* dense_wtab = nullptr);
void vd_launch_dof_grade_dense(hipStream_t s, const uint8_t* L_in, const uint8_t* R_in, const float* dn, int eh, int ew, int H, int W,
                               const vd_finish_consts& fc, const vd_dev_work* w, float focal_override, int use_override,
                               int bar_width, int bar_side, uint8_t* L_out, uint8_t* R_out, const float* wtab);
#define VD_D4_WTAB_FLOATS (4 * 31 * 32)
bool vd_launch_sharp_fit(hipStream_t s, const uint8_t* gL, const uint8_t* gR, const vd3d_render_params& p, const vd_finish_consts& fc, uint8_t* out);
void vd_launch_sharp_mux(hipStream_t s, const uint8_t* gL, const uint8_t* gR, const vd3d_render_params& p,
                         const vd_finish_consts& fc, uint8_t* out, int presharp_pitch = 0, bool identity_fit = false);
void vd_launch_stream_copy(hipStream_t s, const void* src, void* dst, size_t bytes);
void vd_launch_interp_planes(hipStream_t s, const float* src, int C, int ih, int iw, float* dst, int oh, int ow, int premult);
void vd_launch_torch_math_aten(hipStream_t s, int op, const float* x, double p, float* out, long long n, int threads);
void vd_launch_torch_math(hipStream_t s, int op, const float* x, float p, float* out, long long n);
void vd_launch_blank_eye(hipStream_t s, const uint8_t* src, int h, int w, const vd_dev_work* wk, uint8_t* dst);

bool vd_launch_preview(hipStream_t s, int type, const uint8_t* L, const uint8_t* R, int h, int w, uint8_t* out);
int vd_launch_depth_prep(hipStream_t s, const uint8_t* frames, int B, int H, int W, int th, int tw, const float mean[3],
                         const float stdv[3], int dtype, void* out_nhwc, int form);
#define VD_PIL_KMAX 24
struct vd_pil_axis {
  int n_in = 0, n_out = 0;
  int taps = 0;
  int span[6] = {0, 0, 0, 0, 0, 0};
  int* dev = nullptr;
};
int vd_pil_axis_build(vd_pil_axis* a, int n_in, int n_out, hipError_t* herr);
void vd_pil_lut_fill(const float mean[3], const float stdv[3], float* lut768);
bool vd_pil_plan(const vd_pil_axis* aw, const vd_pil_axis* ah, int B, int* by_out);
bool vd_launch_pil_resample(hipStream_t s, const uint8_t* frames, int B, int H, int W, const vd_pil_axis* aw, const vd_pil_axis* ah, int epi,
                            const float* lut_dev, void* out);
long long vd_gemm_x3_weight_bytes(int N, int K, int mode);
bool vd_launch_gemm_x3_pack_w(hipStream_t s, const float* W, int N, int K, void* img, int mode);
bool vd_launch_gemm_x3(hipStream_t s, const float* X, long long M, int K, const void* wimg, int N, const float* bias, int epilogue, float* Y, int mode);
long long vd_conv3x3_x2_weight_bytes(int Cin, int Cout);
bool vd_launch_conv3x3_x2_pack(hipStream_t s, const float* W, int Cin, int Cout, void* img);
bool vd_launch_conv3x3_x2(hipStream_t s, const float* X, int B, int H, int W, int Cin, const void* wimg, int Cout, float* Y);
long long vd_conv3x3_x3_weight_bytes(int Cin, int Cout);
bool vd_launch_conv3x3_x3_pack(hipStream_t s, const float* W, int Cin, int Cout, void* img);
bool vd_launch_conv3x3_x3(hipStream_t s, const float* X, int B, int H, int W, int Cin, const void* wimg, int Cout, float* Y);
long long vd_conv3x3_s2_x3_weight_bytes(int Cin, int Cout);
bool vd_launch_conv3x3_s2_x3_pack(hipStream_t s, const float* W, int Cin, int Cout, void* img);
bool vd_launch_conv3x3_s2_x3(hipStream_t s, const float* X, int B, int H, int W, int Cin, const void* wimg, int Cout, float* Y);
long long vd_conv3x3_s1_x2_weight_bytes(int Cin, int Cout);
bool vd_launch_conv3x3_s1_x2_pack(hipStream_t s, const float* W, int Cin, int Cout, void* img);
bool vd_launch_conv3x3_s1_x2(hipStream_t s, const float* X, int B, int H, int W, int Cin, const void* wimg, int Cout, float* Y);
long long vd_conv3x3_s2_x2_weight_bytes(int Cin, int Cout);
bool vd_launch_conv3x3_s2_x2_pack(hipStream_t s, const float* W, int Cin, int Cout, void* img);
bool vd_launch_conv3x3_s2_x2(hipStream_t s, const float* X, int B, int H, int W, int Cin, const void* wimg, int Cout, float* Y);
long long vd_dpt_head_conv_weight_bytes(int Cin, int Cout);
bool vd_launch_dpt_head_conv_pack(hipStream_t s, const float* W, int Cin, int Cout, void* img);
bool vd_dpt_head_conv_shape_ok(int B, int ih, int iw, int oh, int ow, int Cin, int Cout, bool tail);
bool vd_launch_dpt_head_conv_f32(hipStream_t s, const float* x, const float* b_in, int B, int ih, int iw, int oh, int ow, int Cin, const void* wimg, int Cout,
                                 const float* b2, const float* w3, float b3, float scale, float* out);
long long vd_conv_ifn_weight_bytes(int kind, int Cin, int Cout);
bool vd_launch_conv_ifn_pack(hipStream_t s, int kind, const float* W, int Cin, int Cout, void* img);
bool vd_launch_conv_ifn(hipStream_t s, int kind, const float* X, int B, int H, int W, int x_stride, int Cin, const void* wimg, const float* bias,
                        const float* slope, int Cout, const float* R, int r_stride, float* Y, int y_stride, int y_offset);
void vd_launch_rife_warp_pack(hipStream_t s, const float* X, const float* S, int first, int N, int h, int w, int Hp, int Wp, int scale, float* out);
void vd_launch_rife_update(hipStream_t s, const float* T, int t_stride, int first, int N, int Hp, int Wp, int scale, float* S);
void vd_launch_rife_blend(hipStream_t s, const float* X, const float* S, int N, int h, int w, int Hp, int Wp, float* out);
long long vd_attn_x3_workspace_bytes(int B, int T, int H, int D, int mode);
bool vd_launch_attn_x3(hipStream_t s, const float* qkv, int B, int T, int H, int D, float scale, void* ws, float* out, int mode);
bool vd_launch_attn_f32(hipStream_t s, const float* qkv, int B, int T, int H, int D, float scale, float* out, int form);
bool vd_launch_add_layernorm(hipStream_t s, int dtype, const void* x, const void* y, const void* gamma, const void* beta, float eps,
                             long long rows, int cols, void* out_sum, void* out_norm);
bool vd_launch_upsample_bilinear_nhwc(hipStream_t s, int dtype, const void* in, void* out, int B, int ih, int iw, int oh, int ow, int C);
bool vd_launch_bias_act_f32(hipStream_t s, const float* y, const float* bias, const float* r1, const float* r2, int relu, long long n_pix, int C,
                            float* out, float* relu_out);
bool vd_launch_upsample_bilinear_bias_nhwc_f32(hipStream_t s, const float* in, const float* bias, float* out, int B, int ih, int iw, int oh, int ow, int C);
bool vd_launch_head_tail_f32(hipStream_t s, const float* y, const float* b2, const float* w3, float b3, float scale, long long n_pix, int C, float* out);
bool vd_launch_depth_to_space_bias_f32(hipStream_t s, const float* y, const float* bias, int B, int H, int W, int f, int C, float* out);
bool vd_launch_patchify_f32(hipStream_t s, const float* x, int B, int th, int tw, int p, float* out);
bool vd_launch_depth_handoff(hipStream_t s, const float* pred, int B, int ph, int pw, int H, int W, int invert, uint32_t* mm,
                             uint8_t* out, int form);

#define VD_PCLIP_NR 6
#define VD_PCLIP_WS_WORDS (4 * VD_PCLIP_NR * 256)
bool vd_launch_tile_gather(hipStream_t s, const uint8_t* frames, long long pitch, long long fstride, int B, int H, int W, const int32_t* origins,
                           int n, int ch, int cw, int chs, int cws, uint8_t* out);
void vd_launch_tile_blend(hipStream_t s, const float* pool, const long long* pred_off, const int32_t* tab, const float* wpool, int B, int H, int W,
                          int tile, int core, float* out);
void vd_launch_pclip_u8(hipStream_t s, const float* planes, int B, long long n, const uint32_t rank[VD_PCLIP_NR], float g_lo, float g_hi, int invert,
                        uint32_t* ws, uint8_t* out, float* lohi);

struct vd_lb_ws;
void vd_lb_free(vd_lb_ws* w);
bool vd_lb_size_ok(int B, int H, int W);
hipError_t vd_lb_state_reset(vd_lb_ws** ws, hipStream_t s);
hipError_t vd_lb_state_export(vd_lb_ws** ws, hipStream_t s, vd3d_letterbox_state* out, uint32_t* prev_hist64, uint8_t* prev_gray_dev, long long gray_cap);
hipError_t vd_lb_state_import(vd_lb_ws** ws, hipStream_t s, const vd3d_letterbox_state* in, const uint32_t* prev_hist64, const uint8_t* prev_gray_dev);
hipError_t vd_lb_stats(vd_lb_ws** ws, hipStream_t s, const uint8_t* frames, int B, int H, int W, int chain, float* row_mean, float* row_var,
                       uint32_t* row_sat, uint8_t* gray, uint32_t* hist, unsigned long long* mad, float* fmean);
hipError_t vd_lb_stats_commit(vd_lb_ws** ws, hipStream_t s, const uint8_t* gray, const uint32_t* hist, int B, int H, int W);
hipError_t vd_lb_canny(vd_lb_ws** ws, hipStream_t s, const uint8_t* gray, int B, int H, int W, int low, int high, uint8_t* edges, int32_t* rowcnt);
hipError_t vd_lb_hysteresis(vd_lb_ws** ws, hipStream_t s, const uint8_t* cls, int B, int H, int W, uint8_t* edges, int32_t* rowcnt);
hipError_t vd_lb_track(vd_lb_ws** ws, hipStream_t s, const uint8_t* frames, int B, int H, int W, const vd3d_letterbox_params* p, int32_t* out_bars);
hipError_t vd_lb_fill(vd_lb_ws** ws, hipStream_t s, const uint8_t* depth, int B, int H, int W, const int32_t* bars_dev, int bars_stride, uint8_t* out);

bool vd_launch_finish_fused(hipStream_t s, const uint8_t* L, const uint8_t* R, const float* dn, int eh, int ew,
                            const vd3d_render_params& p, const vd_finish_consts& fc, const vd_dev_work* w, float focal,
                            int use_override, int bar_w, int bar_s, uint8_t* out, int dense, const float* w2_dev);

bool vd_launch_conv3x3_c64_f16(hipStream_t s, const void* x, int H, int W, const void* wfrag, const float* bias, const float* slope_or_null, void* y);
void vd_launch_conv3x3_head_f16(hipStream_t s, const void* x, int H, int W, const float* w27, const float* bias, const float* slope_or_null, void* y);
void vd_launch_esr_tail_f32(hipStream_t s, const void* t, const void* x, int H, int W, int r, float* out);
bool vd_launch_conv3x3_dense_f16(hipStream_t s, const void* x, int H, int W, int x_stride, int Cin, const void* wfrag, const float* bias, int Cout,
                                 float slope, float alpha, const void* r1, int r1_stride, float beta, const void* r2, int r2_stride, int up2,
                                 void* y, int y_stride, int y_offset);
void vd_launch_nhwc_f16_to_planar3_f32(hipStream_t s, const void* t, int H, int W, float* out);
void vd_launch_nv12_to_bgr(hipStream_t s, const uint8_t* y, const uint8_t* uv, int h, int w, long long y_pitch, long long uv_pitch, uint8_t* out);
void vd_launch_bgr_to_nv12(hipStream_t s, const uint8_t* bgr, int h, int w, uint8_t* y, uint8_t* uv, long long y_pitch, long long uv_pitch);
bool vd_launch_preview_heatmap(hipStream_t s, int type, const float* shift, int h, int w, const uint8_t* lut_dev, uint32_t* mm, uint8_t* out);
void vd_launch_preview_arrows(hipStream_t s, const uint8_t* left, const float* shift, int h, int w, uint8_t* out);
bool vd_launch_resize_cubic_u8(hipStream_t s, const uint8_t* src, int sh, int sw, int cn, uint8_t* dst, int dh, int dw);
bool vd_launch_resize_area_u8(hipStream_t s, const uint8_t* src, int sh, int sw, uint8_t* dst, int dh, int dw);
void vd_launch_resize_linear_u8(hipStream_t s, const uint8_t* src, int sh, int sw, uint8_t* dst, int dh, int dw);
bool vd_launch_rife_pre(hipStream_t s, int dtype, const uint8_t* f1, const uint8_t* f2, int h, int w, int hwc, void* out);
void vd_launch_rife_post(hipStream_t s, const float* pred, int h, int w, int hwc, uint8_t* dst);
bool vd_launch_esr_pre(hipStream_t s, int dtype, const uint8_t* src, long long pitch, int h, int w, int hwc, void* out);
void vd_launch_esr_post(hipStream_t s, const float* pred, int h, int w, int hwc, int cy, int cx, int ch, int cw, uint8_t* dst, long long pitch);
void vd_launch_add_weighted_u8(hipStream_t s, const uint8_t* a, float alpha, const uint8_t* b, float beta, float gamma, long long n, uint8_t* out);

void vd_launch_heal(hipStream_t s, const float* warped, const float* orig, const float* edge_or_null, int H, int W, float hs, float* out);
```

visiondepth3d_amd/depth.py:

```python
from __future__ import annotations

import json
import os
import zlib

import numpy as np
import torch
import torch.nn.functional as F

_DA_S = dict(arch="da", hidden=384, layers=12, heads=6, out_indices=[9, 10, 11, 12], neck=[48, 96, 192, 384], fusion=64, head=32)
_DA_B = dict(arch="da", hidden=768, layers=12, heads=12, out_indices=[9, 10, 11, 12], neck=[96, 192, 384, 768], fusion=128, head=32)
_DA_L = dict(arch="da", hidden=1024, layers=24, heads=16, out_indices=[21, 22, 23, 24], neck=[256, 512, 1024, 1024], fusion=256, head=32)
MODEL_ZOO = {
    "depth-anything-v2-small": _DA_S, "depth-anything-v2-base": _DA_B, "depth-anything-v2-large": _DA_L,
    "depth-anything-v1-small": _DA_S, "depth-anything-v1-base": _DA_B, "depth-anything-v1-large": _DA_L,
    "distill-any-depth-small": _DA_S, "distill-any-depth-large": _DA_L,
    "dpt-large": dict(arch="dpt", hidden=1024, layers=24, heads=16, out_indices=[5, 11, 17, 23], neck=[256, 512, 1024, 1024], fusion=256),
}
IMAGENET_MEAN = (0.485, 0.456, 0.406)
IMAGENET_STD = (0.229, 0.224, 0.225)
PROCESSORS = {
    "da": dict(size=(518, 518), keep_aspect_ratio=True, multiple=14, mean=IMAGENET_MEAN, std=IMAGENET_STD),
    "dpt": dict(size=(384, 384), keep_aspect_ratio=False, multiple=1, mean=(0.5, 0.5, 0.5), std=(0.5, 0.5, 0.5)),
}
# ... 204 lines not shown
            tn.set_filename(os.path.join(_tunable_scratch_dir(), "tunableop_results.csv"))
            self.tuned_gemm = bool(tn.read_file(table))
            if not self.tuned_gemm:
                tn.enable(False)
        except Exception:
            self.tuned_gemm = False

    @classmethod
    def from_pretrained(cls, path: str, device="cuda", dtype=torch.float32, **kw) -> "DepthPipe":
        from transformers import AutoModelForDepthEstimation
        if not os.path.isdir(path):
            raise FileNotFoundError(f"{path}: not a local checkpoint folder (this build environment has no network)")
        model = AutoModelForDepthEstimation.from_pretrained(path, local_files_only=True)
        proc = dict(PROCESSORS["da" if type(model).__name__ == "DepthAnythingForDepthEstimation" else "dpt"])
        pc = os.path.join(path, "preprocessor_config.json")
        if os.path.exists(pc):
            with open(pc) as f:
                j = json.load(f)
            sz = j.get("size") or {}
            if isinstance(sz, dict) and "height" in sz:
                proc["size"] = (int(sz["height"]), int(sz["width"]))
            elif isinstance(sz, int):
                proc["size"] = (sz, sz)
            proc["keep_aspect_ratio"] = bool(j.get("keep_aspect_ratio", proc["keep_aspect_ratio"]))
            proc["multiple"] = int(j.get("ensure_multiple_of", proc["multiple"]))
            if j.get("image_mean") is not None:
                proc["mean"] = tuple(float(v) for v in j["image_mean"])
            if j.get("image_std") is not None:
                proc["std"] = tuple(float(v) for v in j["image_std"])
            if int(j.get("resample", 3)) != 3:
                raise NotImplementedError("image processors other than bicubic (PIL resample 3) are not built")
        return cls(os.path.basename(os.path.normpath(path)), device=device, dtype=dtype, model=model, processor=proc, **kw)

    def resize_target(self, h: int, w: int):
        return dpt_resize_target(h, w, self.proc["size"], self.proc["multiple"], self.proc["keep_aspect_ratio"])

    def _cache_position_embeddings(self):
        emb = self.model.backbone.embeddings
        orig = emb.interpolate_pos_encoding
        cache = {}

        def cached(embeddings, height, width):
            key = (int(height), int(width), embeddings.dtype, embeddings.shape[1])
            if key not in cache:
                cache[key] = orig(embeddings, height, width).detach()
            return cache[key]

        emb.interpolate_pos_encoding = cached

    def _patch_dpt_upsampling(self):
        R = self.renderer
        f32 = self.dtype == torch.float32 and os.environ.get("VD3D_NECK_GLUE", "1") != "0"
        CL = torch.channels_last
        sc = self.self_contained

        def up(x, size):
            if x.dtype in (torch.bfloat16, torch.float32) and x.shape[1] % 8 == 0 and x.is_contiguous(memory_format=CL):
                return R.upsample_bilinear(x, size)
            return F.interpolate(x, size=size, mode="bilinear", align_corners=True)

        conv_img = {}

        def conv_x2(m, x):
            if (self.gemm != "fp16x2" or self.conv is not None or not f32 or m.kernel_size != (3, 3) or m.stride != (1, 1) or m.padding != (1, 1) or m.dilation != (1, 1) or m.groups != 1
                    or x.dtype != torch.float32):
                return None
            key = id(m)
            if key not in conv_img:
                conv_img[key] = R.conv3x3_x2_pack(m.weight)
            if conv_img[key] is None:
                return None
            if x.shape[0] * ((x.shape[2] + 15) // 16) * ((x.shape[3] + 31) // 32) < 256:
                return None
            return R.conv3x3_x2(x.contiguous(memory_format=CL), conv_img[key], m.out_channels)

        conv3_img = {}
        names = {id(m): n for n, m in self.model.named_modules()}
        cm = self.conv
        tile_fn, min_tiles = ("conv3x3_s1_x2", CONV_X2_MIN_TILES) if cm == "fp16x2" else ("conv3x3_x3", CONV_X3_MIN_TILES)

        def tile_conv(x, img, n):
            return getattr(R, tile_fn)(x, img, n)

        def conv_x3(m, x):
            if (cm is None or not f32 or m.kernel_size != (3, 3) or m.stride != (1, 1) or m.padding != (1, 1) or m.dilation != (1, 1) or m.groups != 1
                    or x.dtype != torch.float32):
                return None
            key = id(m)
            if key not in conv3_img:
                conv3_img[key] = getattr(R, tile_fn + "_pack")(m.weight)
            if conv3_img[key] is None:
                if sc:
                    raise NotImplementedError(f"self_contained=True: {names[key]}: vd3d_{tile_fn} does not build {m.in_channels} -> {m.out_channels} channels")
                self.conv_routes[names[key]] = ("library", f"shape not built: {m.in_channels} -> {m.out_channels} channels")
                return None
            if sc:
                self.conv_routes[names[key]] = (cm, "self-contained")
                return tile_conv(x.contiguous(memory_format=CL), conv3_img[key], m.out_channels)
            if cm == "fp16x2":
                tiles = ((x.shape[2] + 7) // 8) * ((x.shape[3] + 31) // 32)
            else:
                tiles = x.shape[0] * ((x.shape[2] + 7) // 8) * ((x.shape[3] + 31) // 32)
            if tiles < min_tiles:
                self.conv_routes[names[key]] = ("library", f"size rule: {tiles} tiles < {min_tiles}")
                return None
            self.conv_routes[names[key]] = (cm, f"{tiles} tiles")
            return tile_conv(x.contiguous(memory_format=CL), conv3_img[key], m.out_channels)

        if cm is not None and f32:
            for m in self.model.neck.convs:
                if sc and m.bias is not None:
                    raise NotImplementedError(f"self_contained=True: {names[id(m)]} has a bias (the stock neck convolutions have none) -- not built")
                if m.bias is None:
                    def neck_conv_fwd(x, m=m):
                        y = conv_x3(m, x)
                        if y is None and sc:
                            raise NotImplementedError(f"self_contained=True: {names[id(m)]} is not a float32 3 x 3 / stride 1 / padding 1 convolution -- not built")
                        return F.conv2d(x, m.weight, None, m.stride, m.padding, m.dilation, m.groups) if y is None else y
                    m.forward = neck_conv_fwd

        def conv_nb(m, x):
            y = conv_x2(m, x)
            if y is None:
                y = conv_x3(m, x)
            if y is None and sc:
                raise NotImplementedError(f"self_contained=True: {names[id(m)]} is not a float32 3 x 3 / stride 1 / padding 1 convolution -- not built")
            if y is None:
                y = F.conv2d(x, m.weight, None, m.stride, m.padding, m.dilation, m.groups).contiguous(memory_format=CL)
            if self._flop_count is not None:
                self._flop_count[0] += 2.0 * y.numel() / y.shape[0] * (m.in_channels // m.groups) * m.kernel_size[0] * m.kernel_size[1]
            return y

        gemm_img = {}

        def conv1x1_x3(m, x):
            if m.kernel_size != (1, 1) or m.stride != (1, 1) or m.padding != (0, 0) or m.groups != 1 or m.in_channels % 16 or x.dtype != torch.float32:
                raise NotImplementedError(f"self_contained=True: {names[id(m)]} is not a float32 1 x 1 convolution with C_in a multiple of 16 -- not built")
            if id(m) not in gemm_img:
                gemm_img[id(m)] = R.gemm_x3_pack(m.weight.reshape(m.out_channels, m.in_channels), self.gemm)
            rows = x.contiguous(memory_format=CL).permute(0, 2, 3, 1)
            y = R.linear_x3(rows, gemm_img[id(m)], m.out_channels, None, mode=self.gemm).permute(0, 3, 1, 2)
            self.conv_routes[names[id(m)]] = (self.gemm, "self-contained: vd3d_gemm_x3 over the pixel rows")
            if self._flop_count is not None:
                self._flop_count[0] += 2.0 * y.numel() / y.shape[0] * m.in_channels
            return y

        def res_unit(unit, x, x_relu=None, extra=None, want_relu=False):
            x = x.contiguous(memory_format=CL)
            h = torch.relu(x) if x_relu is None else x_relu
            y = R.bias_act(conv_nb(unit.convolution1, h), unit.convolution1.bias, relu=True)
            y = conv_nb(unit.convolution2, y)
            return R.bias_act(y, unit.convolution2.bias, r1=x, r2=extra, want_relu_copy=want_relu)

        for layer in self.model.neck.fusion_stage.layers:
            def fusion_fwd(hidden_state, residual=None, size=None, layer=layer):
                fused = f32 and hidden_state.dtype == torch.float32 and hidden_state.shape[1] % 4 == 0
                if residual is not None:
                    if hidden_state.shape != residual.shape:
                        residual = F.interpolate(residual, size=(hidden_state.shape[2], hidden_state.shape[3]), mode="bilinear",
                                                 align_corners=False)
                    if fused:
                        hidden_state, hr = res_unit(layer.residual_layer1, residual, extra=hidden_state.contiguous(memory_format=CL), want_relu=True)
                        hidden_state = res_unit(layer.residual_layer2, hidden_state, x_relu=hr)
                    else:
                        hidden_state = layer.residual_layer2(hidden_state + layer.residual_layer1(residual))
                else:
                    hidden_state = res_unit(layer.residual_layer2, hidden_state) if fused else layer.residual_layer2(hidden_state)
                tgt = (2 * hidden_state.shape[2], 2 * hidden_state.shape[3]) if size is None else tuple(size)
                if sc and not (fused and layer.projection.bias is not None):
                    raise NotImplementedError(f"self_contained=True: {names[id(layer)]}: a float32 map with channels in multiples of 4 and a projection with a bias expected")
                if fused and layer.projection.bias is not None:
                    return R.upsample_bilinear_bias((conv1x1_x3 if sc else conv_nb)(layer.projection, hidden_state), tgt, layer.projection.bias)
                return layer.projection(up(hidden_state, tgt))
            layer.forward = fusion_fwd
        if getattr(self, "dpt_vit", False):
            self._patch_dpt_vit_reassemble_head(conv_nb, f32)
            return
        head = self.model.head
        tail_operands = None
        if (f32 and isinstance(head.activation2, torch.nn.ReLU) and head.conv2.out_channels in (16, 32, 64) and head.conv3.kernel_size == (1, 1)
                and head.conv2.bias is not None and head.conv3.bias is not None and head.conv1.bias is not None):
            tail_operands = _head_tail_operands(head.conv3)
        if sc and tail_operands is None:
            raise NotImplementedError("self_contained=True: a depth head other than [conv 3 x 3, up-sampling, conv 3 x 3 -> 16 / 32 / 64, ReLU, conv 1 x 1, ReLU] with biases -- not built")

        head_fused = self.gemm == "f32" and self.conv != "bf16x3" and self.device.type == "cuda"
        head_img = {}

        def head_conv2_image():
            m = head.conv2
            if os.environ.get("VD3D_HEAD_FUSED", "1") == "0":
                return None, "VD3D_HEAD_FUSED=0"
            if m.kernel_size != (3, 3) or m.stride != (1, 1) or m.padding != (1, 1) or m.dilation != (1, 1) or m.groups != 1:
                return None, "not a 3 x 3 / stride 1 / padding 1 convolution"
            try:
                key = (m.weight.data_ptr(), m.weight._version)
            except RuntimeError:
                key = (m.weight.data_ptr(),)
            if head_img.get("key") != key:
                head_img["key"], head_img["img"] = key, (R.dpt_head_conv_pack(m.weight) if m.out_channels == 32 else None)
            if head_img["img"] is None:
                return None, f"shape not built: {m.in_channels} -> {m.out_channels} channels"
            if head.conv1.bias.data_ptr() % 16 or m.bias.data_ptr() % 16 or tail_operands()[0].data_ptr() % 16:
                return None, "a bias or the 1x1 weight is not 16-byte aligned"
            return head_img["img"], f"{m.in_channels} -> {m.out_channels} channels"

        def head_fwd(hidden_states, patch_height, patch_width):
            x = hidden_states[head.head_in_index]
            size = (int(patch_height * head.patch_size), int(patch_width * head.patch_size))
            if tail_operands is not None and x.dtype == torch.float32:
                img = None
                if head_fused:
                    img, why = head_conv2_image()
                    if img is not None and (size[0] < 2 or size[1] < 2):
                        img, why = None, f"output {size[0]} x {size[1]} below 2 x 2"
                    self.conv_routes[names[id(head.conv2)]] = ("f32-fused" if img is not None else "library", why)
                if img is not None:
                    y1 = conv_nb(head.conv1, x.contiguous(memory_format=CL))
                    if self._flop_count is not None:
                        n_out = float(head.conv2.out_channels) * size[0] * size[1]
                        self._flop_count[0] += 2.0 * n_out * head.conv2.in_channels * 9 + 2.0 * n_out
                    w3, b3 = tail_operands()
                    return R.dpt_head_conv(y1, head.conv1.bias, size, img, head.conv2.bias, w3, b3, float(head.max_depth))
                h = R.upsample_bilinear_bias(conv_nb(head.conv1, x.contiguous(memory_format=CL)), size, head.conv1.bias)
                y = conv_nb(head.conv2, h)
                if self._flop_count is not None:
                    self._flop_count[0] += 2.0 * y.numel() / y.shape[0]
                w3, b3 = tail_operands()
                return R.dpt_head_tail(y, head.conv2.bias, w3, b3, float(head.max_depth))
            h = up(head.conv1(x), size)
            h = head.conv3(head.activation1(head.conv2(h)))
            return (head.activation2(h) * head.max_depth).squeeze(dim=1)
        head.forward = head_fwd
        stage = self.model.neck.reassemble_stage

        def reassemble_fwd(hidden_states, patch_height=None, patch_width=None):
            out = []
            for i, hs in enumerate(hidden_states):
                B, _, Cn = hs.shape
                x = hs[:, 1:].reshape(B, patch_height, patch_width, Cn).permute(0, 3, 1, 2)
                out.append(stage.layers[i](x))
            return out
        stage.forward = self._self_contained_reassemble(names) if sc else reassemble_fwd

    def _self_contained_reassemble(self, names):
        R, CL, gm = self.renderer, torch.channels_last, self.gemm
        s2_fn = "conv3x3_s2_x2" if gm == "fp16x2" else "conv3x3_s2_x3"
        stage = self.model.neck.reassemble_stage
        hooks = []
        for lay in stage.layers:
            pm, rz = lay.projection, lay.resize
            if pm.kernel_size != (1, 1) or pm.stride != (1, 1) or pm.padding != (0, 0) or pm.groups != 1 or pm.in_channels % 16:
                raise NotImplementedError(f"self_contained=True: {names[id(pm)]} is not a 1 x 1 convolution with C_in a multiple of 16 -- not built")
            hk = dict(pm=pm, rz=rz, proj=R.gemm_x3_pack(pm.weight.reshape(pm.out_channels, pm.in_channels), gm), kind="identity", img=None)
            if isinstance(rz, torch.nn.ConvTranspose2d):
                if not (rz.kernel_size == rz.stride and rz.kernel_size[0] == rz.kernel_size[1] and rz.padding == (0, 0) and rz.output_padding == (0, 0)
                        and rz.dilation == (1, 1) and rz.groups == 1 and rz.in_channels % 16 == 0 and rz.out_channels % 4 == 0):
                    raise NotImplementedError(f"self_contained=True: {names[id(rz)]}: a ConvTranspose2d with kernel {rz.kernel_size} / stride {rz.stride} / padding "
                                              f"{rz.padding}, {rz.in_channels} -> {rz.out_channels} channels (built: square kernel == stride, no padding, C_in % 16) -- not built")
                hk["kind"], hk["img"] = "ct", R.gemm_x3_pack(conv_transpose_gemm_weight(rz.weight), gm)
            elif isinstance(rz, torch.nn.Conv2d):
                img = None
                if rz.kernel_size == (3, 3) and rz.stride == (2, 2) and rz.padding == (1, 1) and rz.dilation == (1, 1) and rz.groups == 1:
                    img = getattr(R, s2_fn + "_pack")(rz.weight)
                if img is None:
                    raise NotImplementedError(f"self_contained=True: {names[id(rz)]}: a Conv2d with kernel {rz.kernel_size} / stride {rz.stride} / padding {rz.padding}, "
                                              f"{rz.in_channels} -> {rz.out_channels} channels (built: 3 x 3 / stride 2 / padding 1, C_in % 16, C_out % 128 up to 1024) -- not built")
                hk["kind"], hk["img"] = "s2", img
            elif not isinstance(rz, torch.nn.Identity):
                raise NotImplementedError(f"self_contained=True: {names[id(rz)]} ({type(rz).__name__}) is no resize module the mode routes -- not built")
            hooks.append(hk)

        def count(m, y):
            if self._flop_count is not None:
                self._flop_count[0] += 2.0 * y.numel() / y.shape[0] * (m.in_channels // m.groups) * m.kernel_size[0] * m.kernel_size[1]

        def reassemble_fwd(hidden_states, patch_height=None, patch_width=None):
            out = []
            for hk, hs in zip(hooks, hidden_states):
                B, T, _ = hs.shape
                if patch_height is None or patch_width is None:
                    raise ValueError("the DINOv2 reassemble stage needs the patch grid")
                gh, gw = int(patch_height), int(patch_width)
                if gh * gw != T - 1:
                    raise ValueError(f"{T - 1} patch tokens do not form a {gh} x {gw} grid")
                pm, rz = hk["pm"], hk["rz"]
                n = pm.out_channels
                x = R.linear_x3(hs[:, 1:].contiguous(), hk["proj"], n, pm.bias, mode=gm)
                self.conv_routes[names[id(pm)]] = (gm, "self-contained: vd3d_gemm_x3 over the token rows")
                x = x.view(B, gh, gw, n).permute(0, 3, 1, 2)
                count(pm, x)
                if hk["kind"] == "ct":
                    s = rz.kernel_size[0]
                    y = R.linear_x3(x.permute(0, 2, 3, 1), hk["img"], s * s * rz.out_channels, None, mode=gm)
                    x = R.depth_to_space_bias(y.view(B * gh * gw, s * s * rz.out_channels), B, gh, gw, s, rz.bias)
                    self.conv_routes[names[id(rz)]] = (gm, "self-contained: vd3d_gemm_x3 + vd3d_depth_to_space_bias_nhwc_f32")
                    count(rz, x)
                elif hk["kind"] == "s2":
                    x = getattr(R, s2_fn)(x, hk["img"], rz.out_channels)
                    if rz.bias is not None:
                        x = R.bias_act(x, rz.bias)
                    self.conv_routes[names[id(rz)]] = (gm, "self-contained: vd3d_" + s2_fn)
                    count(rz, x)
                out.append(x)
            return out
        return reassemble_fwd

    def _patch_patch_embedding(self):
        R = self.renderer
        pe = self.model.backbone.embeddings.patch_embeddings
        m = pe.projection
        name = next(n for n, mod in self.model.named_modules() if mod is m)
        p = m.kernel_size[0]
        if not (isinstance(m, torch.nn.Conv2d) and m.kernel_size == (p, p) and m.stride == (p, p) and m.padding == (0, 0) and m.dilation == (1, 1) and m.groups == 1
                and m.in_channels == 3 and p <= 64):
            raise NotImplementedError(f"self_contained=True: {name}: a patch embedding other than Conv2d(3, C, kernel_size=p, stride=p), p <= 64 -- not built")
        img = R.gemm_x3_pack(patch_embedding_gemm_weight(m.weight), self.gemm)

        def patch_fwd(pixel_values):
            if pixel_values.dtype != torch.float32 or pixel_values.shape[1] != 3:
                raise NotImplementedError("self_contained=True: the patch embedding takes a float32 [B, 3, th, tw] image")
            rows = R.patchify(pixel_values.contiguous(memory_format=torch.channels_last), p)
            self.conv_routes[name] = (self.gemm, "self-contained: vd3d_patchify_f32 + vd3d_gemm_x3")
            if self._flop_count is not None:
                self._flop_count[0] += 2.0 * rows.shape[1] * m.out_channels * 3 * p * p
            return R.linear_x3(rows, img, m.out_channels, m.bias, mode=self.gemm)
        pe.forward = patch_fwd

    def _patch_dpt_vit_reassemble_head(self, conv_nb, f32):
        R, gm, CL = self.renderer, self.gemm, torch.channels_last
        stage, head = self.model.neck.reassemble_stage, self.model.head
        hooks = []
        for i, lay in enumerate(stage.layers):
            rl, ract = stage.readout_projects[i][0], stage.readout_projects[i][1]
            gelu = isinstance(ract, torch.nn.GELU) and getattr(ract, "approximate", "none") == "none" or type(ract).__name__ == "GELUActivation"
            pw = lay.projection.weight
            hk = dict(readout=(R.gemm_x3_pack(rl.weight, gm), rl.out_features, rl.bias, gelu, ract),
                      proj=(R.gemm_x3_pack(pw.reshape(pw.shape[0], -1), gm), pw.shape[0], lay.projection.bias), resize=lay.resize, ct=None)
            if isinstance(lay.resize, torch.nn.ConvTranspose2d):
                hk["ct"] = (R.gemm_x3_pack(conv_transpose_gemm_weight(lay.resize.weight), gm), lay.resize.kernel_size[0])
            hooks.append(hk)

        def lin(t, img, n, bias, gelu=False, conv=True):
            if conv and self._flop_count is not None:
                self._flop_count[0] += 2.0 * t.numel() / t.shape[0] * n
            return R.linear_x3(t, img, n, bias, gelu=gelu, mode=gm)

        def reassemble_fwd(hidden_states, patch_height=None, patch_width=None):
            out = []
            for hk, hs in zip(hooks, hidden_states):
                B, T, d = hs.shape
                if patch_height is None or patch_width is None:
                    patch_height = patch_width = int((T - 1) ** 0.5)
                gh, gw = int(patch_height), int(patch_width)
                if gh * gw != T - 1:
                    raise ValueError(f"{T - 1} patch tokens do not form a {gh} x {gw} grid")
                img, n, bias, gelu, act = hk["readout"]
                x = torch.cat((hs[:, 1:], hs[:, :1].expand(B, T - 1, d)), -1)
                x = lin(x, img, n, bias, gelu=True, conv=False) if gelu else act(lin(x, img, n, bias, conv=False))
                img, n, bias = hk["proj"]
                x = lin(x, img, n, bias)
                if hk["ct"] is not None:
                    ct_img, s = hk["ct"]
                    y = lin(x, ct_img, s * s * n, None)
                    x = R.depth_to_space_bias(y.view(B * gh * gw, s * s * n), B, gh, gw, s, hk["resize"].bias)
                else:
                    x = x.view(B, gh, gw, n).permute(0, 3, 1, 2)
                    x = hk["resize"](x)
                out.append(x)
            return out
        stage.forward = reassemble_fwd

        if not f32:
            return
        conv1, _, conv2, _, conv3, _ = list(head.head)
        tail_operands = _head_tail_operands(conv3)
        in_index = self.model.config.head_in_index
# ... 373 lines not shown
```

visiondepth3d_amd/render_3d.py:

```python
from __future__ import annotations

import ctypes as C

import numpy as np
import torch

from . import _abi, _lib
from ._abi import DEPTH_BGR_U8, DEPTH_F32, DEPTH_GRAY_U8, DT_BF16, DT_F16, DT_F32, FORMAT_IDS, FrameScalars, LetterboxParams, LetterboxState, RenderParams, ShiftParams, State
from .geometry import aspect_ratios
from .params import reference_aten_threads, render_kwargs_to_params, shift_params_from_kwargs

torch_device = torch.device("cuda" if torch.cuda.is_available() else "cpu")


def _ptr(t: torch.Tensor):
    return C.c_void_p(t.data_ptr())


class Renderer:

    def __init__(self, device: int | torch.device | None = None, private_stream: bool = False, auto_order: bool = True):
        if not torch.cuda.is_available():
            raise RuntimeError("visiondepth3d_amd needs a ROCm GPU (MI355X); there is no CPU path")
        L = _lib.lib()
# ... 840 lines not shown
        return out

    def _conv3x3_x2t_pack(self, st: str, weight: torch.Tensor):
        w = weight.detach().to(self.device, torch.float32).contiguous()
        Cout, Cin, kh, kw = w.shape
        nb = int(getattr(self._L, f"vd3d_conv3x3_{st}_x2_weight_bytes")(Cin, Cout)) if (kh, kw) == (3, 3) else -1
        if nb < 0:
            return None
        img = torch.empty(nb, dtype=torch.uint8, device=self.device)
        self._enter(w, img)
        _lib.check(getattr(self._L, f"vd3d_conv3x3_{st}_x2_pack_weights")(self._ctx, _ptr(w), Cin, Cout, _ptr(img)))
        return img

    def _conv3x3_x2t(self, st: str, x: torch.Tensor, w_image: torch.Tensor, Cout: int) -> torch.Tensor:
        B, Cin, H, W = x.shape
        if x.dtype != torch.float32 or not x.is_contiguous(memory_format=torch.channels_last):
            raise AssertionError(f"conv3x3_{st}_x2: float32 channels_last input")
        Ho, Wo = ((H + 1) // 2, (W + 1) // 2) if st == "s2" else (H, W)
        out = torch.empty((B, int(Cout), Ho, Wo), dtype=torch.float32, device=x.device, memory_format=torch.channels_last)
        self._enter(x, w_image, out)
        _lib.check(getattr(self._L, f"vd3d_conv3x3_{st}_x2")(self._ctx, _ptr(x), B, H, W, Cin, _ptr(w_image), int(Cout), _ptr(out)))
        return out

    def conv3x3_s1_x2_pack(self, weight: torch.Tensor):
        return self._conv3x3_x2t_pack("s1", weight)

    def conv3x3_s1_x2(self, x: torch.Tensor, w_image: torch.Tensor, Cout: int) -> torch.Tensor:
        return self._conv3x3_x2t("s1", x, w_image, Cout)

    def conv3x3_s2_x2_pack(self, weight: torch.Tensor):
        return self._conv3x3_x2t_pack("s2", weight)

    def conv3x3_s2_x2(self, x: torch.Tensor, w_image: torch.Tensor, Cout: int) -> torch.Tensor:
        return self._conv3x3_x2t("s2", x, w_image, Cout)

    def conv_ifn_pack(self, kind: int, weight: torch.Tensor):
        w = weight.detach().to(self.device, torch.float32).contiguous()
        if kind == _abi.IFN_T4S2:
            Cin, Cout, kh, kw = w.shape
            ok = (kh, kw) == (4, 4)
        else:
            Cout, Cin, kh, kw = w.shape
            ok = (kh, kw) == (3, 3)
        nb = int(self._L.vd3d_conv_ifn_weight_bytes(int(kind), Cin, Cout)) if ok else -1
        if nb < 0:
            return None
        img = torch.empty(nb, dtype=torch.uint8, device=self.device)
        self._enter(w, img)
        _lib.check(self._L.vd3d_conv_ifn_pack_weights(self._ctx, int(kind), _ptr(w), Cin, Cout, _ptr(img)))
        return img

    def conv_ifn(self, kind: int, x: torch.Tensor, cin: int, w_image: torch.Tensor, bias: torch.Tensor, slope, cout: int, out: torch.Tensor,
                 out_offset: int = 0, residual=None) -> torch.Tensor:
        for t in (x, out, residual):
            if t is not None and (t.dtype != torch.float32 or t.dim() != 4 or not t.is_contiguous(memory_format=torch.channels_last)):
                raise AssertionError("conv_ifn takes float32 [B,C,H,W] tensors in channels_last memory")
        B, _, H, W = x.shape
        Ho, Wo = {_abi.IFN_K3S1: (H, W), _abi.IFN_K3S2: ((H + 1) // 2, (W + 1) // 2), _abi.IFN_T4S2: (2 * H, 2 * W)}[int(kind)]
        if out.shape[0] != B or tuple(out.shape[2:]) != (Ho, Wo) or (residual is not None and (residual.shape[0] != B or tuple(residual.shape[2:]) != (Ho, Wo))):
            raise AssertionError("conv_ifn: the output and the residual have the kind's output size")
        if bias.dtype != torch.float32 or bias.numel() != cout or (slope is not None and (slope.dtype != torch.float32 or slope.numel() != cout)):
            raise AssertionError("conv_ifn: bias and slope are float32 [cout]")
        self._enter(x, w_image, bias, slope, residual, out)
        _lib.check(self._L.vd3d_conv_ifn(self._ctx, int(kind), _ptr(x), B, H, W, int(x.shape[1]), int(cin), _ptr(w_image), _ptr(bias),
                                         _ptr(slope) if slope is not None else None, int(cout), _ptr(residual) if residual is not None else None,
                                         int(residual.shape[1]) if residual is not None else 0, _ptr(out), int(out.shape[1]), int(out_offset)))
        return out

    @staticmethod
    def _rife_pad(h: int, w: int):
        return (h + 31) // 32 * 32, (w + 31) // 32 * 32

    def rife_warp_pack(self, x6: torch.Tensor, state, scale: int, out: torch.Tensor) -> torch.Tensor:
        N, _, h, w = x6.shape
        Hp, Wp = self._rife_pad(h, w)
        if x6.dtype != torch.float32 or x6.shape[1] != 6 or not x6.is_contiguous() or not out.is_contiguous() or tuple(out.shape) != (N, Hp // scale, Wp // scale, 16):
            raise AssertionError("rife_warp_pack: x6 contiguous float32 [N,6,h,w], out [N,Hp/s,Wp/s,16]")
        if state is not None and (tuple(state.shape) != (N, Hp, Wp, 8) or not state.is_contiguous()):
            raise AssertionError("rife_warp_pack: state is [N,Hp,Wp,8]")
        self._enter(x6, state, out)
        _lib.check(self._L.vd3d_rife_warp_pack(self._ctx, _ptr(x6), _ptr(state) if state is not None else None, N, h, w, int(scale), _ptr(out)))
        return out

    def rife_update(self, t: torch.Tensor, state: torch.Tensor, scale: int, first: bool, h: int, w: int) -> torch.Tensor:
        Hp, Wp = self._rife_pad(h, w)
        N = state.shape[0]
        if tuple(state.shape) != (N, Hp, Wp, 8) or tuple(t.shape[:3]) != (N, Hp // scale, Wp // scale) or not t.is_contiguous() or not state.is_contiguous():
            raise AssertionError("rife_update: t [N,Hp/s,Wp/s,C], state [N,Hp,Wp,8]")
        self._enter(t, state)
        _lib.check(self._L.vd3d_rife_update(self._ctx, _ptr(t), int(t.shape[3]), 1 if first else 0, N, int(h), int(w), int(scale), _ptr(state)))
        return state

    def rife_blend(self, x6: torch.Tensor, state: torch.Tensor, out: torch.Tensor) -> torch.Tensor:
        N, _, h, w = x6.shape
        Hp, Wp = self._rife_pad(h, w)
        if tuple(state.shape) != (N, Hp, Wp, 8) or tuple(out.shape) != (N, 3, h, w) or not out.is_contiguous() or not x6.is_contiguous() or x6.dtype != torch.float32:
            raise AssertionError("rife_blend: x6 [N,6,h,w], state [N,Hp,Wp,8], out [N,3,h,w], float32 contiguous")
        self._enter(x6, state, out)
        _lib.check(self._L.vd3d_rife_blend(self._ctx, _ptr(x6), _ptr(state), N, h, w, _ptr(out)))
        return out

    def upsample_bilinear(self, x: torch.Tensor, size) -> torch.Tensor:
        B, Cc, ih, iw = x.shape
        oh, ow = int(size[0]), int(size[1])
        out = torch.empty((B, Cc, oh, ow), dtype=x.dtype, device=x.device, memory_format=torch.channels_last)
        self._enter(x, out)
        _lib.check(self._L.vd3d_upsample_bilinear_nhwc(self._ctx, self._dt(x.dtype), _ptr(x), _ptr(out), B, ih, iw, oh, ow, Cc))
        return out

    @staticmethod
    def _nhwc_f32(*ts):
        for t in ts:
            if t is not None and not (t.dtype == torch.float32 and t.dim() == 4 and t.is_contiguous(memory_format=torch.channels_last)):
                raise ValueError("float32 channels_last [B,C,h,w] tensors expected")

    def bias_act(self, y, bias=None, r1=None, r2=None, relu=False, want_relu_copy=False):
        self._nhwc_f32(y, r1, r2)
        B, Cc, h, w = y.shape
        ro = torch.empty_like(y) if want_relu_copy else None
        self._enter(y, bias, r1, r2, ro)
        _lib.check(self._L.vd3d_nhwc_bias_act_f32(self._ctx, _ptr(y), _ptr(bias) if bias is not None else None, _ptr(r1) if r1 is not None else None,
                                                  _ptr(r2) if r2 is not None else None, int(bool(relu)), B * h * w, Cc, _ptr(y),
                                                  _ptr(ro) if ro is not None else None))
        return (y, ro) if want_relu_copy else y

    def upsample_bilinear_bias(self, x, size, bias):
        self._nhwc_f32(x)
        B, Cc, ih, iw = x.shape
        oh, ow = int(size[0]), int(size[1])
        out = torch.empty((B, Cc, oh, ow), dtype=x.dtype, device=x.device, memory_format=torch.channels_last)
        self._enter(x, bias, out)
        _lib.check(self._L.vd3d_upsample_bilinear_bias_nhwc_f32(self._ctx, _ptr(x), _ptr(bias), _ptr(out), B, ih, iw, oh, ow, Cc))
        return out

    def dpt_head_tail(self, y, b2, w3, b3: float, scale: float):
        self._nhwc_f32(y)
        B, Cc, h, w = y.shape
        out = torch.empty((B, h, w), dtype=torch.float32, device=y.device)
        self._enter(y, b2, w3, out)
        _lib.check(self._L.vd3d_dpt_head_tail_f32(self._ctx, _ptr(y), _ptr(b2), _ptr(w3), float(b3), float(scale), B * h * w, Cc, _ptr(out)))
        return out

    def dpt_head_conv_pack(self, weight: torch.Tensor):
        w = weight.detach().to(self.device, torch.float32).contiguous()
        Cout, Cin, kh, kw = w.shape
        nb = int(self._L.vd3d_dpt_head_conv_weight_bytes(Cin, Cout)) if (kh, kw) == (3, 3) else -1
        if nb < 0:
            return None
        img = torch.empty(nb, dtype=torch.uint8, device=self.device)
        self._enter(w, img)
        _lib.check(self._L.vd3d_dpt_head_conv_pack_weights(self._ctx, _ptr(w), Cin, Cout, _ptr(img)))
        return img

    def dpt_head_conv(self, x, b_in, size, w_image, b2=None, w3=None, b3: float = 0.0, scale: float = 1.0, Cout=None):
        self._nhwc_f32(x)
        if (b2 is None) != (w3 is None):
            raise ValueError("dpt_head_conv: b2 and w3 go together")
        B, Cin, ih, iw = x.shape
        oh, ow = int(size[0]), int(size[1])
        tail = b2 is not None
        Cout = int(Cout) if Cout is not None else (32 if tail else 64)
        for name, t, n in (("b_in", b_in, Cin), ("b2", b2, Cout), ("w3", w3, Cout)):
            if t is not None and not (t.dtype == torch.float32 and t.is_contiguous() and t.numel() == n):
                raise ValueError(f"dpt_head_conv: {name} must be {n} contiguous float32 values")
        if w_image is None or w_image.numel() != int(self._L.vd3d_dpt_head_conv_weight_bytes(Cin, Cout)):
            raise ValueError(f"dpt_head_conv: the weight image does not belong to a built {Cin} -> {Cout} convolution")
        if tail:
            out = torch.empty((B, oh, ow), dtype=torch.float32, device=x.device)
        else:
            out = torch.empty((B, Cout, oh, ow), dtype=torch.float32, device=x.device, memory_format=torch.channels_last)
        self._enter(x, b_in, w_image, b2, w3, out)
        _lib.check(self._L.vd3d_dpt_head_conv_f32(self._ctx, _ptr(x), _ptr(b_in), B, ih, iw, oh, ow, Cin, _ptr(w_image), Cout,
                                                  _ptr(b2) if tail else None, _ptr(w3) if tail else None, float(b3), float(scale), _ptr(out)))
        return out

    def depth_to_space_bias(self, y, B: int, H: int, W: int, s: int, bias=None):
        P, N = y.shape
        Cc = N // (s * s)
        if y.dtype != torch.float32 or not y.is_contiguous() or P != B * H * W or Cc * s * s != N:
            raise ValueError("y must be contiguous float32 [B*H*W, s*s*C]")
        out = torch.empty((B, Cc, H * s, W * s), dtype=torch.float32, device=y.device, memory_format=torch.channels_last)
        self._enter(y, bias, out)
        _lib.check(self._L.vd3d_depth_to_space_bias_nhwc_f32(self._ctx, _ptr(y), _ptr(bias) if bias is not None else None, int(B), int(H), int(W), int(s), Cc,
                                                             _ptr(out)))
        return out

    def patchify(self, x: torch.Tensor, p: int) -> torch.Tensor:
        B, Cc, th, tw = x.shape
        if x.dtype != torch.float32 or Cc != 3 or not x.permute(0, 2, 3, 1).is_contiguous():
            raise ValueError("patchify: a float32 [B, 3, th, tw] tensor in channels_last memory expected")
        p = int(p)
        if p < 1 or th < p or tw < p:
            raise ValueError(f"patchify: a {th} x {tw} image holds no {p} x {p} patch")
        kp = (3 * p * p + 15) // 16 * 16
        out = torch.empty((B, (th // p) * (tw // p), kp), dtype=torch.float32, device=x.device)
        self._enter(x, out)
        _lib.check(self._L.vd3d_patchify_f32(self._ctx, _ptr(x), B, th, tw, p, _ptr(out)))
        return out

    def detect_black_bars(self, frame_bgr: torch.Tensor):
        f = frame_bgr.to(self.device, torch.uint8).contiguous()
        t, b = C.c_int(), C.c_int()
        self._enter(f)
        _lib.check(self._L.vd3d_detect_black_bars(self._ctx, _ptr(f), f.shape[0], f.shape[1], C.byref(t), C.byref(b)))
        return t.value, b.value

    def debug_planes(self, H, W, eh=None, ew=None):
        ptrs = [C.c_void_p() for _ in range(6)]
        self._L.vd3d_debug_planes(self._ctx, *[C.byref(p) for p in ptrs])
        self.sync()

        def view(ptr, shape, dtype):
            t = torch.empty(shape, dtype=dtype, device=self.device)
            _lib.check(self._L.vd3d_stream_copy(self._ctx, ptr, _ptr(t), t.numel() * t.element_size()))
            return t

        out = {"D": view(ptrs[0], (H, W), torch.float32), "S": view(ptrs[1], (H, W), torch.float32),
               "L": view(ptrs[2], (H, W, 3), torch.uint8), "R": view(ptrs[3], (H, W, 3), torch.uint8)}
        if eh:
            out["rgb_eye"] = view(ptrs[4], (3, eh, ew), torch.float32)
            out["dn"] = view(ptrs[5], (eh, ew), torch.float32)
        self.sync()
        return out


_default: Renderer | None = None


def default_renderer() -> Renderer:
    global _default
    if _default is None:
        _default = Renderer()
    return _default


def frame_to_tensor(frame):
    t = torch.from_numpy(np.ascontiguousarray(frame[..., ::-1])).float().permute(2, 0, 1) / 255.0
    return t.to(torch_device)


def pixel_shift_cuda(frame_tensor, depth_tensor, width, height, fg_shift, mg_shift, bg_shift, return_shift_map=True, **kw):
    p = shift_params_from_kwargs(fg_shift, mg_shift, bg_shift, **kw)
    r = default_renderer()
    res = r.pixel_shift(frame_tensor, depth_tensor, width, height, p, want_shift=bool(return_shift_map))
    if return_shift_map:
        return r.to_host(res[0]).numpy(), r.to_host(res[1]).numpy(), r.to_host(res[2])
    return r.to_host(res[0]).numpy(), r.to_host(res[1]).numpy()


def format_3d_output(left, right, fmt):
    r = default_renderer()
    out = r.format_3d_output(torch.from_numpy(np.ascontiguousarray(left)), torch.from_numpy(np.ascontiguousarray(right)), fmt)
    return r.to_host(out).numpy()


def generate_anaglyph_3d(left_frame, right_frame):
    return format_3d_output(left_frame, right_frame, "Red-Cyan Anaglyph")


def heal_missing_pixels(warped_frame, warped_depth, original_frame, edge_mask, heal_strength=0.5):
    return default_renderer().heal_missing_pixels(warped_frame, original_frame, edge_mask, heal_strength)


def render_clip(frames, depths, **kw):
    return render_pairs(zip(frames, depths), **kw)


def render_pairs(pairs, *, renderer: Renderer | None = None, target_ratio=16 / 9, keep_on_device=False,
                 blank_frames=None, start_frame_idx=0, skip_first=True, batch=8, aten_sum_threads=None, **kw):
    r = renderer or default_renderer()
    blank = set(blank_frames or ()) if kw.get("skip_blank_frames") else set()
    kw["aten_sum_threads"] = reference_aten_threads() if aten_sum_threads is None else int(aten_sum_threads)
    it = iter(pairs)
    if skip_first and next(it, None) is None:
        return
    if int(batch) > 1 and hasattr(r, "shard2_p1_batch"):
        yield from _render_pairs_batched(r, it, int(batch), target_ratio, keep_on_device, blank, start_frame_idx, kw)
        return
    params = None
    for idx, (f, d) in enumerate(it):
        if params is None:
            params = render_kwargs_to_params(int(f.shape[1]), int(f.shape[0]), target_ratio=target_ratio, **kw)
            r.new_clip()
        ft = f if torch.is_tensor(f) else torch.from_numpy(np.ascontiguousarray(f))
        dt = d if torch.is_tensor(d) else torch.from_numpy(np.ascontiguousarray(d))
        out = r.render_frame(ft.to(r.device, non_blocking=True), dt.to(r.device, non_blocking=True), params,
                             blank=(start_frame_idx + idx) in blank)
        if getattr(r, "_private", False):
            r.ordered_after()
        yield out if keep_on_device else out.cpu().numpy()


def _render_pairs_batched(r, it, B, target_ratio, keep_on_device, blank, start_frame_idx, kw):
    from .sharded import ChunkSharder, HipChunkBackend
    sets, params, pending, idx0 = None, None, [], 0

    def drain(step):
        sh, outs = step
        for j, o in enumerate(outs):
            r.wait_pixels(sh.slot_base + j)
            yield o if keep_on_device else o.cpu().numpy()
    k = 0
    try:
        while True:
            chunk = []
            for f, d in it:
                chunk.append((f, d))
                if len(chunk) == B:
                    break
            if not chunk:
                break
            if params is None:
                f0 = chunk[0][0]
                params = render_kwargs_to_params(int(f0.shape[1]), int(f0.shape[0]), target_ratio=target_ratio, **kw)
                r.new_clip()
                be = HipChunkBackend(r, params)
                first = ChunkSharder(be, 0, 1, B)
                sets = [first, ChunkSharder(be, 0, 1, B, slot_base=B, twin_of=first)]
                r.set_pixel_overlap(2)
            T = lambda a: (a if torch.is_tensor(a) else torch.from_numpy(np.ascontiguousarray(a))).to(r.device, non_blocking=True)
            fl, dl = [T(f) for f, _ in chunk], [T(d) for _, d in chunk]
            flags = [(start_frame_idx + idx0 + j) in blank for j in range(len(chunk))] if blank else None
            sh = sets[k % 2]
            outs = sh.render_step(fl, dl, n_valid=len(chunk), blank=flags, first_step=(k == 0), more_steps=True)
            pending.append((sh, outs))
            if len(pending) == 2:
                yield from drain(pending.pop(0))
# ... 14 lines not shown
```

Baseline: 144.5 stereo-pairs/s.

## Fuse last fusion-layer upsample into head conv1 loader and add persistent conv form

The last DPT fusion layer now hands its un-upsampled projection output straight to head.conv1. A new fused kernel performs the x2 bilinear upsample and bias add inside its loader, so the upsampled 128-channel map is never written to and re-read from memory. A persistent-workgroup variant of the head conv kernel (form 2) is also added, with a selectable form and grid size. This adds complexity in the model glue through handed-through state, plus extra validation paths.

```diff
diff --git a/include/vd3d.h b/include/vd3d.h
--- a/include/vd3d.h
+++ b/include/vd3d.h
@@ -293,6 +293,8 @@
 int vd3d_dpt_head_conv_pack_weights(vd3d_ctx* ctx, const float* W, int Cin, int Cout, void* image);
 int vd3d_dpt_head_conv_f32(vd3d_ctx* ctx, const float* x, const float* b_in, int B, int ih, int iw, int oh, int ow, int Cin, const void* w_image, int Cout,
                            const float* b2_or_null, const float* w3_or_null, float b3, float scale, float* out);
+int vd3d_dpt_head_conv_f32_form(vd3d_ctx* ctx, int form, int workgroups, const float* x, const float* b_in, int B, int ih, int iw, int oh, int ow, int Cin,
+                                const void* w_image, int Cout, const float* b2_or_null, const float* w3_or_null, float b3, float scale, float* out);
 
 int vd3d_depth_to_space_bias_nhwc_f32(vd3d_ctx* ctx, const float* y, const float* bias_or_null, int B, int H, int W, int s, int C, float* out);
 
diff --git a/visiondepth3d_amd/_lib.py b/visiondepth3d_amd/_lib.py
--- a/visiondepth3d_amd/_lib.py
+++ b/visiondepth3d_amd/_lib.py
@@ -15,7 +15,7 @@
     "vd3d_state_reset", "vd3d_state_new_clip", "vd3d_state_export", "vd3d_state_import", "vd3d_state_planes",
     "vd3d_last_scalars", "vd3d_pixel_shift", "vd3d_render_frame", "vd3d_render_frame_blank", "vd3d_depth_handoff", "vd3d_depth_handoff_form", "vd3d_heal_missing_pixels", "vd3d_preview_heatmap", "vd3d_preview_arrows", "vd3d_conv3x3_c64_f16", "vd3d_conv3x3_head_f16", "vd3d_esr_tail_f32", "vd3d_conv3x3_dense_f16", "vd3d_nhwc_f16_to_planar3_f32", "vd3d_nv12_to_bgr", "vd3d_bgr_to_nv12", "vd3d_resize_cubic_u8", "vd3d_resize_area_u8", "vd3d_resize_linear_u8", "vd3d_format_3d_output", "vd3d_esr_preprocess", "vd3d_esr_postprocess", "vd3d_add_weighted_u8", "vd3d_rife_preprocess", "vd3d_rife_postprocess",
     "vd3d_shard_begin", "vd3d_shard_pixels", "vd3d_shard_pixels_blank", "vd3d_tdf_plane_export", "vd3d_tdf_plane_import", "vd3d_set_pixel_overlap", "vd3d_join_pixels", "vd3d_wait_pixels", "vd3d_finish_frame", "vd3d_quantiles",
-    "vd3d_subject_depth", "vd3d_shard2_p0", "vd3d_shard2_set_crops", "vd3d_shard2_p1", "vd3d_shard2_p1_batch", "vd3d_shard2_r1", "vd3d_shard2_p3", "vd3d_shard2_p3_batch", "vd3d_shard2_r2", "vd3d_depth_preprocess", "vd3d_depth_preprocess_form", "vd3d_resize_pil_bicubic_u8", "vd3d_depth_preprocess_pil", "vd3d_tile_gather_cubic_u8", "vd3d_tile_blend_f32", "vd3d_depth_normalize_pclip_u8", "vd3d_letterbox_stats", "vd3d_canny_u8", "vd3d_canny_hysteresis_u8", "vd3d_letterbox_track", "vd3d_letterbox_state_reset", "vd3d_letterbox_state_export", "vd3d_letterbox_state_import", "vd3d_depth_letterbox_fill_u8", "vd3d_add_layernorm", "vd3d_gemm_x3_weight_bytes", "vd3d_gemm_x3_pack_weights", "vd3d_gemm_x3", "vd3d_attention_x3_workspace_bytes", "vd3d_attention_x3", "vd3d_attention_f32", "vd3d_attention_f32_form", "vd3d_conv3x3_x2_weight_bytes", "vd3d_conv3x3_x2_pack_weights", "vd3d_conv3x3_x2", "vd3d_conv3x3_x3_weight_bytes", "vd3d_conv3x3_x3_pack_weights", "vd3d_conv3x3_x3", "vd3d_conv3x3_s2_x3_weight_bytes", "vd3d_conv3x3_s2_x3_pack_weights", "vd3d_conv3x3_s2_x3", "vd3d_conv3x3_s1_x2_weight_bytes", "vd3d_conv3x3_s1_x2_pack_weights", "vd3d_conv3x3_s1_x2", "vd3d_conv3x3_s2_x2_weight_bytes", "vd3d_conv3x3_s2_x2_pack_weights", "vd3d_conv3x3_s2_x2", "vd3d_conv_ifn_weight_bytes", "vd3d_conv_ifn_pack_weights", "vd3d_conv_ifn", "vd3d_rife_warp_pack", "vd3d_rife_update", "vd3d_rife_blend", "vd3d_upsample_bilinear_nhwc", "vd3d_nhwc_bias_act_f32", "vd3d_upsample_bilinear_bias_nhwc_f32", "vd3d_dpt_head_tail_f32", "vd3d_dpt_head_conv_weight_bytes", "vd3d_dpt_head_conv_pack_weights", "vd3d_dpt_head_conv_f32", "vd3d_depth_to_space_bias_nhwc_f32", "vd3d_patchify_f32", "vd3d_preview_image", "vd3d_detect_black_bars", "vd3d_stream_copy", "vd3d_torch_math", "vd3d_torch_math_aten", "vd3d_debug_gaussian_kernel1d", "vd3d_debug_exp_torch", "vd3d_set_profiling", "vd3d_last_stage_ms", "vd3d_stage_calls",
+    "vd3d_subject_depth", "vd3d_shard2_p0", "vd3d_shard2_set_crops", "vd3d_shard2_p1", "vd3d_shard2_p1_batch", "vd3d_shard2_r1", "vd3d_shard2_p3", "vd3d_shard2_p3_batch", "vd3d_shard2_r2", "vd3d_depth_preprocess", "vd3d_depth_preprocess_form", "vd3d_resize_pil_bicubic_u8", "vd3d_depth_preprocess_pil", "vd3d_tile_gather_cubic_u8", "vd3d_tile_blend_f32", "vd3d_depth_normalize_pclip_u8", "vd3d_letterbox_stats", "vd3d_canny_u8", "vd3d_canny_hysteresis_u8", "vd3d_letterbox_track", "vd3d_letterbox_state_reset", "vd3d_letterbox_state_export", "vd3d_letterbox_state_import", "vd3d_depth_letterbox_fill_u8", "vd3d_add_layernorm", "vd3d_gemm_x3_weight_bytes", "vd3d_gemm_x3_pack_weights", "vd3d_gemm_x3", "vd3d_attention_x3_workspace_bytes", "vd3d_attention_x3", "vd3d_attention_f32", "vd3d_attention_f32_form", "vd3d_conv3x3_x2_weight_bytes", "vd3d_conv3x3_x2_pack_weights", "vd3d_conv3x3_x2", "vd3d_conv3x3_x3_weight_bytes", "vd3d_conv3x3_x3_pack_weights", "vd3d_conv3x3_x3", "vd3d_conv3x3_s2_x3_weight_bytes", "vd3d_conv3x3_s2_x3_pack_weights", "vd3d_conv3x3_s2_x3", "vd3d_conv3x3_s1_x2_weight_bytes", "vd3d_conv3x3_s1_x2_pack_weights", "vd3d_conv3x3_s1_x2", "vd3d_conv3x3_s2_x2_weight_bytes", "vd3d_conv3x3_s2_x2_pack_weights", "vd3d_conv3x3_s2_x2", "vd3d_conv_ifn_weight_bytes", "vd3d_conv_ifn_pack_weights", "vd3d_conv_ifn", "vd3d_rife_warp_pack", "vd3d_rife_update", "vd3d_rife_blend", "vd3d_upsample_bilinear_nhwc", "vd3d_nhwc_bias_act_f32", "vd3d_upsample_bilinear_bias_nhwc_f32", "vd3d_dpt_head_tail_f32", "vd3d_dpt_head_conv_weight_bytes", "vd3d_dpt_head_conv_pack_weights", "vd3d_dpt_head_conv_f32", "vd3d_dpt_head_conv_f32_form", "vd3d_depth_to_space_bias_nhwc_f32", "vd3d_patchify_f32", "vd3d_preview_image", "vd3d_detect_black_bars", "vd3d_stream_copy", "vd3d_torch_math", "vd3d_torch_math_aten", "vd3d_debug_gaussian_kernel1d", "vd3d_debug_exp_torch", "vd3d_set_profiling", "vd3d_last_stage_ms", "vd3d_stage_calls",
     "vd3d_debug_planes", "vd3d_debug_tune",
 )
 
@@ -155,6 +155,7 @@
     L.vd3d_dpt_head_conv_weight_bytes.restype = C.c_int64
     L.vd3d_dpt_head_conv_pack_weights.argtypes = [vp, vp, i32, i32, vp]
     L.vd3d_dpt_head_conv_f32.argtypes = [vp, vp, vp, i32, i32, i32, i32, i32, i32, vp, i32, vp, vp, C.c_float, C.c_float, vp]
+    L.vd3d_dpt_head_conv_f32_form.argtypes = [vp, i32, i32, vp, vp, i32, i32, i32, i32, i32, i32, vp, i32, vp, vp, C.c_float, C.c_float, vp]
     L.vd3d_depth_to_space_bias_nhwc_f32.argtypes = [vp, vp, vp, i32, i32, i32, i32, i32, vp]
     L.vd3d_patchify_f32.argtypes = [vp, vp, i32, i32, i32, i32, vp]
     L.vd3d_preview_image.argtypes = [vp, i32, vp, vp, i32, i32, vp]
diff --git a/visiondepth3d_amd/csrc/vd3d_api.hip b/visiondepth3d_amd/csrc/vd3d_api.hip
--- a/visiondepth3d_amd/csrc/vd3d_api.hip
+++ b/visiondepth3d_amd/csrc/vd3d_api.hip
@@ -1869,9 +1869,11 @@
   HIPCHK(hipGetLastError());
   return 0;
 }
-VD3D_EXPORT int vd3d_dpt_head_conv_f32(vd3d_ctx* c, const float* x, const float* b_in, int B, int ih, int iw, int oh, int ow, int Cin, const void* w_image, int Cout,
-                                       const float* b2_or_null, const float* w3_or_null, float b3, float scale, float* out) {
+VD3D_EXPORT int vd3d_dpt_head_conv_f32_form(vd3d_ctx* c, int form, int workgroups, const float* x, const float* b_in, int B, int ih, int iw, int oh, int ow, int Cin,
+                                            const void* w_image, int Cout, const float* b2_or_null, const float* w3_or_null, float b3, float scale, float* out) {
   if (!c || !x || !b_in || !w_image || !out || (b2_or_null == nullptr) != (w3_or_null == nullptr)) return set_err(VD3D_E_INVALID, "bad argument");
+  if (form < 0 || form > 2) return set_err(VD3D_E_INVALID, "dpt_head_conv: form %d is not 0 (choose), 1 (one workgroup per tile) or 2 (persistent)", form);
+  if (workgroups < 0) return set_err(VD3D_E_INVALID, "dpt_head_conv: workgroups %d is negative (0 = choose)", workgroups);
   const bool tail = b2_or_null != nullptr;
   if (!vd_dpt_head_conv_shape_ok(B, ih, iw, oh, ow, Cin, Cout, tail))
     return set_err(VD3D_E_UNSUPPORTED, "dpt_head_conv: shape not built: %d -> %d channels %s, batch %d, %d x %d -> %d x %d (built: 32 | 64 | 128 -> 32 with the tail, "
@@ -1880,10 +1882,14 @@
       (reinterpret_cast<uintptr_t>(out) & (tail ? 3 : 15)) || (tail && ((reinterpret_cast<uintptr_t>(b2_or_null) & 15) || (reinterpret_cast<uintptr_t>(w3_or_null) & 15))))
     return set_err(VD3D_E_UNSUPPORTED, "dpt_head_conv: x, b_in, the weight image, b2, w3 and a plain output must be 16-byte aligned (the tail's output 4-byte)");
   HIPCHK(hipSetDevice(c->device));
-  if (!vd_launch_dpt_head_conv_f32(c->stream, x, b_in, B, ih, iw, oh, ow, Cin, w_image, Cout, b2_or_null, w3_or_null, b3, scale, out))
+  if (!vd_launch_dpt_head_conv_f32(c->stream, x, b_in, B, ih, iw, oh, ow, Cin, w_image, Cout, b2_or_null, w3_or_null, b3, scale, out, form, workgroups))
     return set_err(VD3D_E_HIP, "dpt_head_conv: the dynamic LDS opt-in or the launch failed");
   HIPCHK(hipGetLastError());
   return 0;
+}
+VD3D_EXPORT int vd3d_dpt_head_conv_f32(vd3d_ctx* c, const float* x, const float* b_in, int B, int ih, int iw, int oh, int ow, int Cin, const void* w_image, int Cout,
+                                       const float* b2_or_null, const float* w3_or_null, float b3, float scale, float* out) {
+  return vd3d_dpt_head_conv_f32_form(c, 0, 0, x, b_in, B, ih, iw, oh, ow, Cin, w_image, Cout, b2_or_null, w3_or_null, b3, scale, out);
 }
 VD3D_EXPORT int vd3d_depth_to_space_bias_nhwc_f32(vd3d_ctx* c, const float* y, const float* bias_or_null, int B, int H, int W, int s, int C, float* out) {
   if (!c || !y || !out || B < 1 || H < 1 || W < 1 || s < 1 || C < 1) return set_err(VD3D_E_INVALID, "bad argument");
diff --git a/visiondepth3d_amd/csrc/vd3d_conv_head.hip b/visiondepth3d_amd/csrc/vd3d_conv_head.hip
--- a/visiondepth3d_amd/csrc/vd3d_conv_head.hip
+++ b/visiondepth3d_amd/csrc/vd3d_conv_head.hip
@@ -165,6 +165,203 @@
   }
 }
 
+template <int C_IN, int C_OUT, bool TAIL>
+__global__ __launch_bounds__(CH_NT) void k_conv3x3_up_p_f32(const float* __restrict__ X, const float* __restrict__ bin, const float* __restrict__ Wimg,
+                                                            const float* __restrict__ b2, const float* __restrict__ w3, float* __restrict__ out, vd_ch_args a,
+                                                            int ntiles, int total) {
+  constexpr int NM = C_OUT / 32, NCHUNK = C_IN / 16, WBUF = ch_w_buf(C_OUT), WLDS = ch_w_lds(C_OUT), W_ITEMS = WBUF / 16, W_ITERS = (W_ITEMS + CH_NT - 1) / CH_NT;
+  constexpr bool STAG = NM == 1, PRE = NM == 1;
+  constexpr int W_HALF = (W_ITERS + 1) / 2;
+  static_assert(NCHUNK >= 2 && NCHUNK % 2 == 0, "buffer parity = chunk parity across tiles");
+  extern __shared__ __attribute__((aligned(16))) uint8_t ch_smem[];
+  const int G = (int)gridDim.x, g0 = (int)blockIdx.x;
+  const int tid = threadIdx.x, lane = tid & 63, wave = __builtin_amdgcn_readfirstlane(tid >> 6);
+  const int li = lane & 31, kh = lane >> 5, hi = wave >> 2;
+
+  int o00[CH_ITERS], o01[CH_ITERS], o10[CH_ITERS], o11[CH_ITERS], dst[CH_ITERS];
+  float ly1[CH_ITERS], lx1[CH_ITERS];
+  bool inside[CH_ITERS];
+  const float* xb = X;
+#pragma unroll
+  for (int it = 0; it < CH_ITERS; ++it) dst[it] = ((tid & 3) * CH_PLANE + ((it * CH_NT + tid) >> 2)) * 16;
+  auto setup = [&](int t) {
+    const int b = t / ntiles, tile = t - b * ntiles;
+    const int tyi = tile / a.ntx, txi = tile - tyi * a.ntx;
+    const int y0 = tyi * CH_TH, x0 = txi * CH_TW;
+    xb = X + (size_t)b * a.ih * a.iw * C_IN;
+#pragma unroll
+    for (int it = 0; it < CH_ITERS; ++it) {
+      const int i = it * CH_NT + tid, pix = i >> 2, q = i & 3;
+      const int py = pix / CH_PW, px = pix - py * CH_PW;
+      const int gy = y0 - 1 + py, gx = x0 - 1 + px;
+      inside[it] = i < CH_ITEMS && gy >= 0 && gy < a.oh && gx >= 0 && gx < a.ow;
+      const int cy = inside[it] ? gy : 0, cx = inside[it] ? gx : 0;
+      const float fy = a.sh * (float)cy, fx = a.sw * (float)cx;
+      const int yy0 = (int)fy, xx0 = (int)fx;
+      const int yy1 = yy0 + (yy0 < a.ih - 1 ? 1 : 0), xx1 = xx0 + (xx0 < a.iw - 1 ? 1 : 0);
+      ly1[it] = fy - (float)yy0; lx1[it] = fx - (float)xx0;
+      o00[it] = (yy0 * a.iw + xx0) * C_IN + q * 4; o01[it] = (yy0 * a.iw + xx1) * C_IN + q * 4;
+      o10[it] = (yy1 * a.iw + xx0) * C_IN + q * 4; o11[it] = (yy1 * a.iw + xx1) * C_IN + q * 4;
+    }
+  };
+  ch_f4 p00[CH_ITERS], p01[CH_ITERS], p10[CH_ITERS], p11[CH_ITERS], wv[W_ITERS], bq, ov;
+  auto load_item = [&](int it, int chunk) {
+    p00[it] = *reinterpret_cast<const ch_f4*>(xb + o00[it] + chunk * 16); p01[it] = *reinterpret_cast<const ch_f4*>(xb + o01[it] + chunk * 16);
+    p10[it] = *reinterpret_cast<const ch_f4*>(xb + o10[it] + chunk * 16); p11[it] = *reinterpret_cast<const ch_f4*>(xb + o11[it] + chunk * 16);
+  };
+  auto load_bq = [&](int chunk) { bq = *reinterpret_cast<const ch_f4*>(bin + chunk * 16 + (tid & 3) * 4); };
+  auto load_w = [&](int chunk) {
+#pragma unroll
+    for (int p = 0; p < W_ITERS; ++p)
+      wv[p] = *reinterpret_cast<const ch_f4*>(Wimg + (size_t)chunk * (WBUF / 4) + (p * CH_NT + tid < W_ITEMS ? p * CH_NT + tid : W_ITEMS - 1) * 4);
+  };
+  auto load = [&](int chunk) {
+    load_bq(chunk);
+#pragma unroll
+    for (int it = 0; it < CH_ITERS; ++it) load_item(it, chunk);
+    load_w(chunk);
+  };
+  auto interp_half = [&](int it, int half, int buf) {
+    asm volatile("" : "+v"(p00[it]), "+v"(p01[it]), "+v"(p10[it]), "+v"(p11[it]));
+    const float l_y1 = ly1[it], l_y0 = 1.f - l_y1, l_x1 = lx1[it], l_x0 = 1.f - l_x1;
+    if (half == 0) {
+      ov.x = (l_y0 * (l_x0 * p00[it].x + l_x1 * p01[it].x) + l_y1 * (l_x0 * p10[it].x + l_x1 * p11[it].x)) + bq.x;
+      ov.y = (l_y0 * (l_x0 * p00[it].y + l_x1 * p01[it].y) + l_y1 * (l_x0 * p10[it].y + l_x1 * p11[it].y)) + bq.y;
+    } else {
+      ov.z = (l_y0 * (l_x0 * p00[it].z + l_x1 * p01[it].z) + l_y1 * (l_x0 * p10[it].z + l_x1 * p11[it].z)) + bq.z;
+      ov.w = (l_y0 * (l_x0 * p00[it].w + l_x1 * p01[it].w) + l_y1 * (l_x0 * p10[it].w + l_x1 * p11[it].w)) + bq.w;
+      if (!inside[it]) ov = ch_f4{0.f, 0.f, 0.f, 0.f};
+      *reinterpret_cast<ch_f4*>(ch_smem + buf * CH_X_BUF + dst[it]) = ov;
+    }
+  };
+  auto put_w = [&](int buf, int p0, int p1) {
+#pragma unroll
+    for (int p = p0; p < p1; ++p) *reinterpret_cast<ch_f4*>(ch_smem + 2 * CH_X_BUF + buf * WLDS + (p * CH_NT + tid) * 16) = wv[p];
+  };
+
+  x3_f16 tot[NM];
+#pragma unroll
+  for (int m = 0; m < NM; ++m)
+#pragma unroll
+    for (int r = 0; r < 16; ++r) tot[m][r] = 0.f;
+  auto epilogue = [&](int t) {
+    const int b = t / ntiles, tile = t - b * ntiles;
+    const int tyi = tile / a.ntx, txi = tile - tyi * a.ntx;
+    const int y = tyi * CH_TH + wave, x = txi * CH_TW + li;
+    const bool live = y < a.oh && x < a.ow;
+    const size_t pix = ((size_t)b * a.oh + (live ? y : 0)) * a.ow + (live ? x : 0);
+    if constexpr (TAIL) {
+      float s = 0.f;
+#pragma unroll
+      for (int g4 = 0; g4 < 4; ++g4) {
+        const ch_f4 bb = *reinterpret_cast<const ch_f4*>(b2 + 8 * g4 + 4 * kh), ww = *reinterpret_cast<const ch_f4*>(w3 + 8 * g4 + 4 * kh);
+        s = vd_fma(fmaxf(tot[0][4 * g4] + bb.x, 0.f), ww.x, s);
+        s = vd_fma(fmaxf(tot[0][4 * g4 + 1] + bb.y, 0.f), ww.y, s);
+        s = vd_fma(fmaxf(tot[0][4 * g4 + 2] + bb.z, 0.f), ww.z, s);
+        s = vd_fma(fmaxf(tot[0][4 * g4 + 3] + bb.w, 0.f), ww.w, s);
+      }
+      s += __shfl_xor(s, 32, 64);
+      if (live && kh == 0) out[pix] = fmaxf(s + a.b3, 0.f) * a.scale;
+    } else {
+      if (live) {
+#pragma unroll
+        for (int m = 0; m < NM; ++m)
+#pragma unroll
+          for (int g4 = 0; g4 < 4; ++g4)
+            *reinterpret_cast<ch_f4*>(out + pix * C_OUT + m * 32 + 8 * g4 + 4 * kh) =
+                ch_f4{tot[m][4 * g4], tot[m][4 * g4 + 1], tot[m][4 * g4 + 2], tot[m][4 * g4 + 3]};
+      }
+    }
+  };
+
+  setup(g0);
+  load(0);
+#pragma unroll
+  for (int it = 0; it < CH_ITERS; ++it) { interp_half(it, 0, 0); interp_half(it, 1, 0); }
+  put_w(0, 0, W_ITERS);
+  __syncthreads();
+
+  const int fx_base = (kh * CH_PLANE + (wave + 1) * CH_PW + li + 1) * 16;
+  const int fw_base = 2 * CH_X_BUF + (kh * C_OUT + li) * 16;
+#pragma unroll 1
+  for (int t = g0; t < total; t += G) {
+    const bool more = t + G < total;
+#pragma unroll 1
+    for (int chunk = 0; chunk < NCHUNK; ++chunk) {
+      const int cur = chunk & 1, nxt = cur ^ 1;
+      const int nchunk = chunk + 1 < NCHUNK ? chunk + 1 : 0;
+      const uint8_t* xs = ch_smem + cur * CH_X_BUF + fx_base;
+      const uint8_t* ws = ch_smem + cur * WLDS + fw_base;
+      x3_f16 acc[2][NM];
+#pragma unroll
+      for (int m = 0; m < NM; ++m)
+#pragma unroll
+        for (int r = 0; r < 16; ++r) acc[0][m][r] = acc[1][m][r] = 0.f;
+      ch_f4 bfr[2], afr[2][NM];
+      auto frags = [&](int gi, int set) {
+        const int tap = gi >> 1, g = gi & 1, dy = tap / 3 - 1, dx = tap - (tap / 3) * 3 - 1;
+        bfr[set] = *reinterpret_cast<const ch_f4*>(xs + (2 * g * CH_PLANE + dy * CH_PW + dx) * 16);
+#pragma unroll
+        for (int m = 0; m < NM; ++m) afr[set][m] = *reinterpret_cast<const ch_f4*>(ws + ((tap * 4 + 2 * g) * C_OUT + m * 32) * 16);
+      };
+      if constexpr (PRE) frags(0, 0);
+#pragma unroll
+      for (int gi = 0; gi < 18; ++gi) {
+        const int set = PRE ? (gi & 1) : 0;
+        if constexpr (PRE) { if (gi + 1 < 18) frags(gi + 1, set ^ 1); }
+        else frags(gi, 0);
+#pragma unroll
+        for (int m = 0; m < NM; ++m) acc[0][m] = __builtin_amdgcn_mfma_f32_32x32x2f32(afr[set][m].x, bfr[set].x, acc[0][m], 0, 0, 0);
+#pragma unroll
+        for (int m = 0; m < NM; ++m) acc[1][m] = __builtin_amdgcn_mfma_f32_32x32x2f32(afr[set][m].y, bfr[set].y, acc[1][m], 0, 0, 0);
+#pragma unroll
+        for (int m = 0; m < NM; ++m) acc[0][m] = __builtin_amdgcn_mfma_f32_32x32x2f32(afr[set][m].z, bfr[set].z, acc[0][m], 0, 0, 0);
+#pragma unroll
+        for (int m = 0; m < NM; ++m) acc[1][m] = __builtin_amdgcn_mfma_f32_32x32x2f32(afr[set][m].w, bfr[set].w, acc[1][m], 0, 0, 0);
+        if (gi < 2 && chunk == 0 && gi == hi) {
+          if (t != g0) epilogue(t - G);
+#pragma unroll
+          for (int m = 0; m < NM; ++m)
+#pragma unroll
+            for (int r = 0; r < 16; ++r) tot[m][r] = 0.f;
+        }
+        if constexpr (STAG) {
+          if ((gi & 1) == hi) {
+            const int j = gi >> 1;
+            if (j == 0) load_bq(nchunk);
+            if (j < 3) load_item(j, nchunk);
+            if (j == 2) load_w(nchunk);
+            if (j >= 3 && j < 8) interp_half((j - 3) >> 1, (j - 3) & 1, nxt);
+            if (j == 7) put_w(nxt, 0, W_HALF);
+            if (j == 8) {
+              interp_half(2, 1, nxt);
+              put_w(nxt, W_HALF, W_ITERS);
+              if (chunk == NCHUNK - 2 && more) setup(t + G);
+            }
+          }
+        } else {
+          if (gi == 0 || gi == 2 || gi == 4) {
+            __builtin_amdgcn_sched_barrier(0);
+            if (gi == 0) load_bq(nchunk);
+            load_item(gi >> 1, nchunk);
+            if (gi == 4) load_w(nchunk);
+            __builtin_amdgcn_sched_barrier(0);
+          }
+          if ((gi >= 5 && gi <= 10) || gi == 14 || gi == 16) __builtin_amdgcn_sched_barrier(0);
+          if (gi >= 5 && gi <= 10) interp_half((gi - 5) >> 1, (gi - 5) & 1, nxt);
+          if (gi == 14) put_w(nxt, 0, W_HALF);
+          if (gi == 16) put_w(nxt, W_HALF, W_ITERS);
+          if (gi == 17 && chunk == NCHUNK - 2 && more) setup(t + G);
+        }
+      }
+#pragma unroll
+      for (int m = 0; m < NM; ++m) tot[m] = (tot[m] + acc[0][m]) + acc[1][m];
+      __syncthreads();
+    }
+  }
+  epilogue(g0 + ((total - 1 - g0) / G) * G);
+}
+
 __global__ __launch_bounds__(256) void k_conv3x3_up_pack(const float* __restrict__ W, int Cout, int Cin, float4* __restrict__ img) {
   const int t = blockIdx.x * 256 + threadIdx.x;
   const int total = (Cin / 16) * 9 * 4 * Cout;
@@ -196,21 +393,53 @@
   return true;
 }
 
+#define CH_P_MIN_ROUNDS 4
+static int ch_num_cus() {
+  static int n_cu[64] = {};
+  int dev = 0;
+  if (hipGetDevice(&dev) != hipSuccess || dev < 0 || dev >= 64) return 0;
+  if (!n_cu[dev] && hipDeviceGetAttribute(&n_cu[dev], hipDeviceAttributeMultiprocessorCount, dev) != hipSuccess) n_cu[dev] = 0;
+  return n_cu[dev];
+}
+
+#define CH_P_FNS {reinterpret_cast<const void*>(k_conv3x3_up_p_f32<32, 32, true>), ch_lds(32)}, {reinterpret_cast<const void*>(k_conv3x3_up_p_f32<64, 32, true>), ch_lds(32)}, \
+                 {reinterpret_cast<const void*>(k_conv3x3_up_p_f32<128, 32, true>), ch_lds(32)}, {reinterpret_cast<const void*>(k_conv3x3_up_p_f32<128, 64, false>), ch_lds(64)}
+static void ch_launch_p(hipStream_t s, dim3 grid, bool tail, int Cin, const float* x, const float* b_in, const float* wi, const float* b2, const float* w3, float* out,
+                        const vd_ch_args& a, int ntiles, int tot) {
+  if (!tail) hipLaunchKernelGGL((k_conv3x3_up_p_f32<128, 64, false>), grid, dim3(CH_NT), ch_lds(64), s, x, b_in, wi, b2, w3, out, a, ntiles, tot);
+  else if (Cin == 32) hipLaunchKernelGGL((k_conv3x3_up_p_f32<32, 32, true>), grid, dim3(CH_NT), ch_lds(32), s, x, b_in, wi, b2, w3, out, a, ntiles, tot);
+  else if (Cin == 64) hipLaunchKernelGGL((k_conv3x3_up_p_f32<64, 32, true>), grid, dim3(CH_NT), ch_lds(32), s, x, b_in, wi, b2, w3, out, a, ntiles, tot);
+  else hipLaunchKernelGGL((k_conv3x3_up_p_f32<128, 32, true>), grid, dim3(CH_NT), ch_lds(32), s, x, b_in, wi, b2, w3, out, a, ntiles, tot);
+}
+
 bool vd_launch_dpt_head_conv_f32(hipStream_t s, const float* x, const float* b_in, int B, int ih, int iw, int oh, int ow, int Cin, const void* wimg, int Cout,
-                                 const float* b2, const float* w3, float b3, float scale, float* out) {
+                                 const float* b2, const float* w3, float b3, float scale, float* out, int form, int workgroups) {
   const bool tail = b2 != nullptr;
-  if (!vd_dpt_head_conv_shape_ok(B, ih, iw, oh, ow, Cin, Cout, tail)) return false;
+  if (!vd_dpt_head_conv_shape_ok(B, ih, iw, oh, ow, Cin, Cout, tail) || form < 0 || form > 2 || workgroups < 0) return false;
   static bool attr_set[64] = {};
   if (!vd_lds_optin({{reinterpret_cast<const void*>(k_conv3x3_up_f32<32, 32, true>), ch_lds(32)}, {reinterpret_cast<const void*>(k_conv3x3_up_f32<64, 32, true>), ch_lds(32)},
-                     {reinterpret_cast<const void*>(k_conv3x3_up_f32<128, 32, true>), ch_lds(32)}, {reinterpret_cast<const void*>(k_conv3x3_up_f32<128, 64, false>), ch_lds(64)}},
-                    attr_set)) return false;
+                     {reinterpret_cast<const void*>(k_conv3x3_up_f32<128, 32, true>), ch_lds(32)}, {reinterpret_cast<const void*>(k_conv3x3_up_f32<128, 64, false>), ch_lds(64)},
+                     CH_P_FNS}, attr_set)) return false;
   vd_ch_args a;
   a.ih = ih; a.iw = iw; a.oh = oh; a.ow = ow;
   a.sh = (float)(ih - 1) / (float)(oh - 1); a.sw = (float)(iw - 1) / (float)(ow - 1);
   a.ntx = (ow + CH_TW - 1) / CH_TW;
   a.b3 = b3; a.scale = scale;
-  const dim3 grid((unsigned)(a.ntx * ((oh + CH_TH - 1) / CH_TH)), (unsigned)B, 1);
+  const int ntiles = a.ntx * ((oh + CH_TH - 1) / CH_TH);
+  const long long total = (long long)ntiles * B;
   const float* wi = reinterpret_cast<const float*>(wimg);
+  const int n_cu = ch_num_cus();
+  if (form == 0) form = (Cout == 32 && n_cu > 0 && total >= (long long)CH_P_MIN_ROUNDS * n_cu && total < (1ll << 30)) ? 2 : 1;
+  if (form == 2) {
+    if (total >= (1ll << 30)) return false;
+    long long G = workgroups > 0 ? workgroups : (n_cu > 0 ? n_cu : 256);
+    if (G > total) G = total;
+    const dim3 grid((unsigned)G, 1, 1);
+    const int tot = (int)total;
+    ch_launch_p(s, grid, tail, Cin, x, b_in, wi, b2, w3, out, a, ntiles, tot);
+    return true;
+  }
+  const dim3 grid((unsigned)ntiles, (unsigned)B, 1);
   if (!tail) hipLaunchKernelGGL((k_conv3x3_up_f32<128, 64, false>), grid, dim3(CH_NT), ch_lds(64), s, x, b_in, wi, b2, w3, out, a);
   else if (Cin == 32) hipLaunchKernelGGL((k_conv3x3_up_f32<32, 32, true>), grid, dim3(CH_NT), ch_lds(32), s, x, b_in, wi, b2, w3, out, a);
   else if (Cin == 64) hipLaunchKernelGGL((k_conv3x3_up_f32<64, 32, true>), grid, dim3(CH_NT), ch_lds(32), s, x, b_in, wi, b2, w3, out, a);
diff --git a/visiondepth3d_amd/csrc/vd3d_kernels.h b/visiondepth3d_amd/csrc/vd3d_kernels.h
--- a/visiondepth3d_amd/csrc/vd3d_kernels.h
+++ b/visiondepth3d_amd/csrc/vd3d_kernels.h
@@ -225,7 +225,7 @@
 bool vd_launch_dpt_head_conv_pack(hipStream_t s, const float* W, int Cin, int Cout, void* img);
 bool vd_dpt_head_conv_shape_ok(int B, int ih, int iw, int oh, int ow, int Cin, int Cout, bool tail);
 bool vd_launch_dpt_head_conv_f32(hipStream_t s, const float* x, const float* b_in, int B, int ih, int iw, int oh, int ow, int Cin, const void* wimg, int Cout,
-                                 const float* b2, const float* w3, float b3, float scale, float* out);
+                                 const float* b2, const float* w3, float b3, float scale, float* out, int form = 0, int workgroups = 0);
 long long vd_conv_ifn_weight_bytes(int kind, int Cin, int Cout);
 bool vd_launch_conv_ifn_pack(hipStream_t s, int kind, const float* W, int Cin, int Cout, void* img);
 bool vd_launch_conv_ifn(hipStream_t s, int kind, const float* X, int B, int H, int W, int x_stride, int Cin, const void* wimg, const float* bias,
diff --git a/visiondepth3d_amd/depth.py b/visiondepth3d_amd/depth.py
--- a/visiondepth3d_amd/depth.py
+++ b/visiondepth3d_amd/depth.py
@@ -380,6 +380,39 @@
             y = conv_nb(unit.convolution2, y)
             return R.bias_act(y, unit.convolution2.bias, r1=x, r2=extra, want_relu_copy=want_relu)
 
+        last_fusion = self.model.neck.fusion_stage.layers[-1]
+        conv1_img, conv1_handed = {}, {}
+
+        def head_conv1_image():
+            head = getattr(self.model, "head", None)
+            m = getattr(head, "conv1", None)
+            if m is None or getattr(self, "dpt_vit", False):
+                return None, "no Depth-Anything head"
+            if not (self.gemm == "f32" and f32 and self.device.type == "cuda"):
+                return None, "not the float32 route on a GPU"
+            if sc or self.conv is not None:
+                return None, "self_contained" if sc else f"conv={self.conv!r} routes it"
+            if os.environ.get("VD3D_HEAD_FUSED", "1") == "0":
+                return None, "VD3D_HEAD_FUSED=0"
+            if tail_operands is None:
+                return None, "a head the float32 glue does not route"
+            if m.kernel_size != (3, 3) or m.stride != (1, 1) or m.padding != (1, 1) or m.dilation != (1, 1) or m.groups != 1:
+                return None, "not a 3 x 3 / stride 1 / padding 1 convolution"
+            if (m.in_channels, m.out_channels) != (128, 64):
+                return None, f"shape not built: {m.in_channels} -> {m.out_channels} channels"
+            pb = last_fusion.projection.bias
+            if pb is None or pb.dtype != torch.float32 or pb.data_ptr() % 16 or not pb.is_contiguous() or last_fusion.projection.out_channels != m.in_channels:
+                return None, "the projection in front has no 16-byte aligned float32 bias"
+            try:
+                key = (m.weight.data_ptr(), m.weight._version)
+            except RuntimeError:
+                key = (m.weight.data_ptr(),)
+            if conv1_img.get("key") != key:
+                conv1_img["key"], conv1_img["img"] = key, R.dpt_head_conv_pack(m.weight)
+            if conv1_img["img"] is None:
+                return None, f"shape not built: {m.in_channels} -> {m.out_channels} channels"
+            return conv1_img["img"], f"{m.in_channels} -> {m.out_channels} channels, the x2 up-sampling in its loader"
+
         for layer in self.model.neck.fusion_stage.layers:
             def fusion_fwd(hidden_state, residual=None, size=None, layer=layer):
                 fused = f32 and hidden_state.dtype == torch.float32 and hidden_state.shape[1] % 4 == 0
@@ -398,7 +431,12 @@
                 if sc and not (fused and layer.projection.bias is not None):
                     raise NotImplementedError(f"self_contained=True: {names[id(layer)]}: a float32 map with channels in multiples of 4 and a projection with a bias expected")
                 if fused and layer.projection.bias is not None:
-                    return R.upsample_bilinear_bias((conv1x1_x3 if sc else conv_nb)(layer.projection, hidden_state), tgt, layer.projection.bias)
+                    y = (conv1x1_x3 if sc else conv_nb)(layer.projection, hidden_state)
+                    conv1_handed.clear()
+                    if layer is last_fusion and size is None and head_conv1_image()[0] is not None:
+                        conv1_handed["y"], conv1_handed["size"] = y, tgt
+                        return y
+                    return R.upsample_bilinear_bias(y, tgt, layer.projection.bias)
                 return layer.projection(up(hidden_state, tgt))
             layer.forward = fusion_fwd
         if getattr(self, "dpt_vit", False):
@@ -433,9 +471,25 @@
                 return None, "a bias or the 1x1 weight is not 16-byte aligned"
             return head_img["img"], f"{m.in_channels} -> {m.out_channels} channels"
 
+        def head_conv1(x):
+            handed, size1 = conv1_handed.pop("y", None), conv1_handed.pop("size", None)
+            img, why = head_conv1_image()
+            if handed is not None:
+                if handed is not x or img is None:
+                    raise RuntimeError("head.conv1: the last fusion layer handed its projection through, but the head was given another map")
+                self.conv_routes[names[id(head.conv1)]] = ("f32-fused", why)
+                if self._flop_count is not None:
+                    self._flop_count[0] += 2.0 * head.conv1.out_channels * size1[0] * size1[1] * head.conv1.in_channels * 9
+                return R.dpt_conv_up(x.contiguous(memory_format=CL), last_fusion.projection.bias, size1, img, head.conv1.out_channels)
+            if self.gemm == "f32" and f32 and not sc and self.conv is None and x.dtype == torch.float32:
+                self.conv_routes[names[id(head.conv1)]] = ("library", why if img is None else "the map in front arrived up-sampled")
+            return conv_nb(head.conv1, x.contiguous(memory_format=CL))
+
         def head_fwd(hidden_states, patch_height, patch_width):
             x = hidden_states[head.head_in_index]
             size = (int(patch_height * head.patch_size), int(patch_width * head.patch_size))
+            if conv1_handed.get("y") is not None and not (tail_operands is not None and x.dtype == torch.float32):
+                raise RuntimeError("head.conv1: the fused loader was chosen for a head that does not take it")
             if tail_operands is not None and x.dtype == torch.float32:
                 img = None
                 if head_fused:
@@ -444,13 +498,13 @@
                         img, why = None, f"output {size[0]} x {size[1]} below 2 x 2"
                     self.conv_routes[names[id(head.conv2)]] = ("f32-fused" if img is not None else "library", why)
                 if img is not None:
-                    y1 = conv_nb(head.conv1, x.contiguous(memory_format=CL))
+                    y1 = head_conv1(x)
                     if self._flop_count is not None:
                         n_out = float(head.conv2.out_channels) * size[0] * size[1]
                         self._flop_count[0] += 2.0 * n_out * head.conv2.in_channels * 9 + 2.0 * n_out
                     w3, b3 = tail_operands()
                     return R.dpt_head_conv(y1, head.conv1.bias, size, img, head.conv2.bias, w3, b3, float(head.max_depth))
-                h = R.upsample_bilinear_bias(conv_nb(head.conv1, x.contiguous(memory_format=CL)), size, head.conv1.bias)
+                h = R.upsample_bilinear_bias(head_conv1(x), size, head.conv1.bias)
                 y = conv_nb(head.conv2, h)
                 if self._flop_count is not None:
                     self._flop_count[0] += 2.0 * y.numel() / y.shape[0]
diff --git a/visiondepth3d_amd/render_3d.py b/visiondepth3d_amd/render_3d.py
--- a/visiondepth3d_amd/render_3d.py
+++ b/visiondepth3d_amd/render_3d.py
@@ -1016,7 +1016,10 @@
         _lib.check(self._L.vd3d_dpt_head_conv_pack_weights(self._ctx, _ptr(w), Cin, Cout, _ptr(img)))
         return img
 
-    def dpt_head_conv(self, x, b_in, size, w_image, b2=None, w3=None, b3: float = 0.0, scale: float = 1.0, Cout=None):
+    def dpt_head_conv(self, x, b_in, size, w_image, b2=None, w3=None, b3: float = 0.0, scale: float = 1.0, Cout=None, form: int = 0, workgroups: int = 0, out=None):
+        return self._dpt_head_conv(x, b_in, size, w_image, b2, w3, b3, scale, Cout, form, workgroups, out)
+
+    def _dpt_head_conv(self, x, b_in, size, w_image, b2, w3, b3, scale, Cout, form, workgroups, out):
         self._nhwc_f32(x)
         if (b2 is None) != (w3 is None):
             raise ValueError("dpt_head_conv: b2 and w3 go together")
@@ -1029,14 +1032,23 @@
                 raise ValueError(f"dpt_head_conv: {name} must be {n} contiguous float32 values")
         if w_image is None or w_image.numel() != int(self._L.vd3d_dpt_head_conv_weight_bytes(Cin, Cout)):
             raise ValueError(f"dpt_head_conv: the weight image does not belong to a built {Cin} -> {Cout} convolution")
-        if tail:
+        if out is not None:
+            if tail and not (out.dtype == torch.float32 and tuple(out.shape) == (B, oh, ow) and out.is_contiguous() and out.device == x.device):
+                raise ValueError("dpt_head_conv: out must be a contiguous float32 [B, oh, ow] tensor on x's device")
+            if not tail and not (out.dtype == torch.float32 and tuple(out.shape) == (B, Cout, oh, ow) and out.device == x.device
+                                 and out.permute(0, 2, 3, 1).is_contiguous()):
+                raise ValueError("dpt_head_conv: out must be a channels_last float32 [B, Cout, oh, ow] tensor on x's device")
+        elif tail:
             out = torch.empty((B, oh, ow), dtype=torch.float32, device=x.device)
         else:
             out = torch.empty((B, Cout, oh, ow), dtype=torch.float32, device=x.device, memory_format=torch.channels_last)
         self._enter(x, b_in, w_image, b2, w3, out)
-        _lib.check(self._L.vd3d_dpt_head_conv_f32(self._ctx, _ptr(x), _ptr(b_in), B, ih, iw, oh, ow, Cin, _ptr(w_image), Cout,
-                                                  _ptr(b2) if tail else None, _ptr(w3) if tail else None, float(b3), float(scale), _ptr(out)))
-        return out
+        _lib.check(self._L.vd3d_dpt_head_conv_f32_form(self._ctx, int(form), int(workgroups), _ptr(x), _ptr(b_in), B, ih, iw, oh, ow, Cin, _ptr(w_image), Cout,
+                                                       _ptr(b2) if tail else None, _ptr(w3) if tail else None, float(b3), float(scale), _ptr(out)))
+        return out
+
+    def dpt_conv_up(self, x, b_in, size, w_image, Cout: int = 64):
+        return self._dpt_head_conv(x, b_in, size, w_image, None, None, 0.0, 1.0, Cout, 0, 0, None)
 
     def depth_to_space_bias(self, y, B: int, H: int, W: int, s: int, bias=None):
         P, N = y.shape
```

Measured after the change: 145.1 stereo-pairs/s, median of 6. About the same (+0.4%).
